# itailang/SampleNet

Measured on AMD Instinct MI355X. Metric: point-clouds/sec fwd+bwd, Bx1024->64 soft-proj+Chamfer, higher is better.
Workload: dtype f32; 1 GPU; BASELINE configs[1]: SampleNet sampler train step (fwd + simplification/projection losses + bwd), B=32 per GPU, 1024->64 points, K=8, bottleneck 128; no optimizer step; batch_per_gpu=32, global_batch=32, n_in=1024, n_out=64, group_size=8, parallelism=dp1, rccl_ranks=0, grad_allreduce=none, execution=whole step replayed as one hipGraph

## Files before the change

### include/samplenet_hip_internal.h

```cpp
#ifndef SAMPLENET_HIP_INTERNAL_H
#define SAMPLENET_HIP_INTERNAL_H

#include "samplenet_hip.h"

#ifdef __cplusplus
extern "C" {
#endif

int sn_sampler_loss_forward(int nproj, const float *proj, const float *lsimp, const float *temperature,
                            float alpha, float lmbda, float min_sigma, float *loss, sn_stream_t stream);
int sn_sampler_loss_backward(int nproj, const float *grad_loss, const float *temperature, float alpha, float lmbda,
                             float min_sigma, float *grad_proj, float *grad_lsimp, float *grad_T, sn_stream_t stream);

int sn_pairscan_colmin_splits(int B, int N, int M);
int sn_pairscan_forward_partial(int B, int N, int M, int K, const float *P, int p_layout, const float *Q, int q_layout,
                                int *knn_idx, float *dist_q, int *idx_q, float *proj, int proj_layout,
                                const float *temperature, float min_sigma, void *workspace, long long workspace_bytes,
                                sn_stream_t stream);
int sn_pairscan_forward_partial_fc(int B, int N, int M, int K, const float *P, int p_layout, const float *fc_z,
                                   const float *fc_scale, const float *fc_shift, const float *fc_w, const float *fc_bias,
                                   int Kfc, float *q_out, int *knn_idx, float *dist_q, int *idx_q, float *proj,
                                   int proj_layout, const float *temperature, float min_sigma, void *workspace,
                                   long long workspace_bytes, sn_stream_t stream);
int sn_sampler_step_loss_forward(int B, int M, int N, int G, const float *dist_q, const void *colmin_ws, const float *proj,
                                 const float *temperature, float alpha, float lmbda, float weight, float min_sigma,
                                 float *dist_p, int *idx_p, int *argmax1, float *partial, float *loss, int defer_value,
                                 sn_stream_t stream);
int sn_sampler_step_loss_forward_direct(int B, int M, int N, const float *dist_q, const float *dist_p, const float *proj,
                                        const float *temperature, float alpha, float lmbda, float weight, float min_sigma,
                                        int *argmax1, float *partial, float *loss, int defer_value, sn_stream_t stream);
int sn_sampler_step_loss_backward(int B, int N, int M, int K, const float *P, int p_layout, const float *Q,
                                  const int *knn_idx, const int *idx_q, const int *idx_p, const int *argmax1,
                                  const float *temperature, float min_sigma, float alpha, float lmbda, float weight,
                                  const float *grad_loss, float *grad_Q, float *gsig_scratch, float *grad_T,
                                  const float *deferred_partial, float *deferred_loss, sn_stream_t stream);
int sn_pairscan_forward_keys(int B, int N, int M, int K, const float *P, int p_layout, float *Q, const float *fc_z,
                             const float *fc_scale, const float *fc_shift, const float *fc_w, const float *fc_bias, int Kfc,
                             int *knn_idx, float *dist_q, int *idx_q, float *proj, int proj_layout, const float *temperature,
                             float min_sigma, void *colmin_keys, float *qpart, void *qmax, sn_stream_t stream);
int sn_sampler_step_loss_keys(int B, int N, int M, int K, const float *P, int p_layout, const float *Q, const int *knn_idx,
                              const int *idx_q, void *colmin_keys, const float *qpart, const void *qmax, int G,
                              const float *temperature, float min_sigma, float alpha, float lmbda, float weight,
                              const float *grad_loss, float *grad_Q, float *gsig_scratch, float *grad_T, float *dpsum,
                              float *loss, sn_stream_t stream, void *deferred_tail, const float *grad_proj,
                              const float *grad_sigma);
int sn_surface_values_keys(int B, int N, int M, int G, const void *colmin_keys, const float *qpart, const void *qmax,
                           const float *temperature, float min_sigma, float weight, const float *y_bcn, float *simp_bnc,
                           float *dpsum, float *values, sn_stream_t stream);
int sn_surface_gather_upstream(int nproj, const float *g_lsimp, const float *g_sigma, const float *g_proj, float *scalars,
                               float *proj_out, sn_stream_t stream);
int sn_conv_stack_set_persist_min_tiles(int tiles);
int sn_fps_set_variant(int v);
int sn_step_tail_bytes(void);
int sn_step_tail_set_error_words(void *tail_blob, const void *fwd_sync, const void *bwd_sync);


int sn_layer_forward_bn(int R, int Ci, int Co, const float *ain, const float *coef_prev, const float *W,
                        const float *bias, float *z, float *stats, const float *gamma, const float *beta,
                        float eps, float momentum, float *running_mean, float *running_var,
                        long long *num_batches_tracked, float *coef, sn_stream_t stream);
int sn_conv_forward_bn_pool(int R, int Ci, int Co, int npts, const float *ain, const float *coef_prev, const float *W,
                            const float *bias, float *z, float *stats, const float *gamma, const float *beta, float eps,
                            float momentum, float *running_mean, float *running_var, long long *num_batches_tracked,
                            float *coef, float *pool_val, int *pool_idx, float *pooled, int *argsel, float *zsel,
                            sn_stream_t stream);
int sn_conv_stack_forward_supported(int B, int N, int nlayers, const int *channels);
long long sn_conv_stack_acc_elems(int nlayers);
int sn_conv_stack_z1_free_supported(int B, int N, int nlayers, const int *channels);
long long sn_conv_stack_acc_sum_elems(int nlayers, const int *channels);
int sn_conv_stack_forward_bn(int B, int N, int nlayers, const int *channels, const float *x, const float *const *W,
                             const float *const *bias, const float *const *gamma, const float *const *beta,
                             float *const *running_mean, float *const *running_var, long long *const *num_batches_tracked,
                             const float *eps, const float *momentum, float *const *z, float *const *coef, long long *acc,
                             float *pool_val, int *pool_idx, float *pooled, int *argsel, float *zsel, sn_stream_t stream);
long long sn_conv_stack_backward_scratch_floats(int B, int N, int nlayers, const int *channels);
int sn_conv_stack_backward(int B, int N, int nlayers, const int *channels, const float *x, const float *const *W,
                           const float *bias0, const float *const *z, const float *const *coef, const float *gsel,
                           const int *argsel, const float *kcoef_top, long long *acc, float *scratch, float *const *dW,
                           float *const *dgamma, float *const *dbeta, float *const *dbias, const void *step_tail,
                           sn_stream_t stream);
int sn_layer_backward(int R, int Ci, int Co, int dz_mode, const float *dy, const float *z, const float *kcoef,
                      const float *gsel, const int *argsel, int npts, const float *W, const float *zprev,
                      const float *coef_prev, float *dyprev, float *stats, float *part, float *dW, float *db,
                      float *prev_dgamma, float *prev_dbeta, float *prev_dbias, float *prev_kcoef, long long prev_bn_rows,
                      sn_stream_t stream);
long long sn_layer_backward_in3_stats_floats(int R, int Ci, int Co);
int sn_layer_backward_in3(int R, int Ci, int Co, const float *dy, const float *z, const float *kcoef, const float *W,
                          const float *zprev, const float *coef_prev, float *stats, float *part, float *dW,
                          float *prev_dgamma, float *prev_dbeta, float *prev_dbias, float *prev_kcoef, const float *x_in,
                          const float *W_in, const float *b_in, float *dW_in, sn_stream_t stream);

int sn_fc_chain_forward_supported(int R, int C0, int H, int nl);
int sn_fc_chain_forward(int R, int C0, int H, int nl, const float *a0, const float *const *W, const float *const *bias,
                        const float *const *gamma, const float *const *beta, float *const *running_mean,
                        float *const *running_var, long long *const *num_batches_tracked, const float *eps,
                        const float *momentum, float *const *z, float *const *coef, float *xbuf, unsigned *sync,
                        sn_stream_t stream);
int sn_fc_chain_forward_pool_supported(int B, int N, int C0, int H, int nl);
int sn_fc_chain_forward_pool(int B, int N, int nconv, long long *acc, const float *pool_val, const int *pool_idx,
                             const float *gamma5, const float *beta5, float *running_mean5, float *running_var5,
                             long long *num_batches_tracked5, float eps5, float momentum5, float *coef5, float *pooled,
                             int *argsel, float *zsel, int H, int nl, const float *const *W, const float *const *bias,
                             const float *const *gamma, const float *const *beta, float *const *running_mean,
                             float *const *running_var, long long *const *num_batches_tracked, const float *eps,
                             const float *momentum, float *const *z, float *const *coef, float *xbuf, unsigned *sync,
                             sn_stream_t stream);
int sn_fc_chain_forward_pool_out_supported(int B, int N, int C0, int H, int nl, int Co);
int sn_fc_chain_forward_pool_out(int B, int N, int nconv, long long *acc, const float *pool_val, const int *pool_idx,
                                 const float *gamma5, const float *beta5, float *running_mean5, float *running_var5,
                                 long long *num_batches_tracked5, float eps5, float momentum5, float *coef5, float *pooled,
                                 int *argsel, float *zsel, int H, int nl, const float *const *W, const float *const *bias,
                                 const float *const *gamma, const float *const *beta, float *const *running_mean,
                                 float *const *running_var, long long *const *num_batches_tracked, const float *eps,
                                 const float *momentum, float *const *z, float *const *coef, float *xbuf, unsigned *sync, int Co,
                                 const float *Wo, const float *bo, const float *gamma_o, const float *beta_o, float *running_mean_o,
                                 float *running_var_o, long long *num_batches_tracked_o, float eps_o, float momentum_o, float *zo,
                                 float *coef_o, float *y, sn_stream_t stream);
int sn_fc_chain_backward_supported(int R, int ns, const int *Co, const int *Ci);
int sn_fc_chain_backward(int R, int ns, const int *Co, const int *Ci, const float *gy, const float *const *W,
                         const float *const *zprev, const float *const *coefprev, const long long *bn_rows,
                         float *const *dgamma, float *const *dbeta, float *const *dbias, float *const *dW, float *db_top,
                         const float *const *aprev, const int *araw, float *gout, float *kout, float *xbuf,
                         unsigned *sync, sn_stream_t stream);
int sn_fc_chain_backward_obn(int R, int ns, const int *Co, const int *Ci, const float *gy, const float *zo, const float *coef_o, int fixed,
                             float *dgamma_o, float *dbeta_o, const float *const *W, const float *const *zprev,
                             const float *const *coefprev, const long long *bn_rows, float *const *dgamma, float *const *dbeta,
                             float *const *dbias, float *const *dW, float *db_top, const float *const *aprev, const int *araw, float *gout,
                             float *kout, float *xbuf, unsigned *sync, sn_stream_t stream);
int sn_bn_batch_stats_twopass(int R, int C, const float *z, const float *gamma, const float *beta, float eps, float momentum,
                              float *running_mean, float *running_var, long long *num_batches_tracked, float *coef,
                              sn_stream_t stream);

int sn_layer_forward_bn_out(int R, int Ci, int Co, const float *ain, const float *coef_prev, const float *W, const float *bias,
                            float *z, const float *gamma, const float *beta, float eps, float momentum, float *running_mean,
                            float *running_var, long long *num_batches_tracked, float *coef, float *y, sn_stream_t stream);
int sn_bn_output_forward(int R, int C, int training, const float *z, const float *gamma, const float *beta, float eps,
                         float momentum, float *running_mean, float *running_var, long long *num_batches_tracked, float *coef,
                         float *y, sn_stream_t stream);
int sn_bn_output_backward(int R, int C, int fixed, const float *gy, const float *z, const float *coef, float *dz, float *dgamma,
                          float *dbeta, sn_stream_t stream);

int sn_pool_backward_bn(int B, int C, long long R, const float *g, const float *pooled, const float *zsel, float *gsel,
                        const float *coef, float *dgamma, float *dbeta, float *dbias, float *kcoef, sn_stream_t stream);

int sn_linear_backward(int R, int Ci, int Co, int dz_mode, const float *dy, const float *z, const float *kcoef,
                       const float *gsel, const int *argsel, int npts, const float *W, const float *zprev,
                       const float *coef_prev, float *dyprev, float *stats, float *part, float *dW, sn_stream_t stream);

int sn_conv_backward_partials(int R, int Ci, int Co, int dz_mode, const float *dy, const float *z, const float *kcoef,
                              const float *gsel, const int *argsel, int npts, const float *W, const float *zprev,
                              const float *coef_prev, float *dyprev, float *stats, float *part, sn_stream_t stream);

int sn_linear_forward_maxpool_supported(int R, int Ci, int Co, int npts);
int sn_linear_forward_maxpool(int R, int Ci, int Co, int npts, const float *ain, const float *coef_prev, const float *W,
                              const float *bias, float *z, unsigned long long *keys, float *pooled, int *argsel, float *zsel,
                              int keys_cleared, sn_stream_t stream);

int sn_linear_forward_maxpool_wide_supported(int R, int Ci, int Co, int npts);
long long sn_linear_forward_maxpool_wide_scratch_bytes(int R, int Ci, int Co, int npts);
int sn_linear_forward_maxpool_wide(int R, int Ci, int Co, int npts, const float *ain, const float *coef_prev, const float *W,
                                   const float *bias, float *z, void *scratch, float *pooled, int *argsel, float *zsel,
                                   void *wplanes, int planes_ready, sn_stream_t stream);
int sn_pool_dgrad_sparse_supported(int B, int npts, int Ci, int Co);
// ... 112 lines not shown
```

### samplenet_amd/_lib.py

```python
import ctypes
import os

import torch

_HERE = os.path.dirname(os.path.abspath(__file__))
LIB_PATH = os.environ.get("SAMPLENET_AMD_LIB") or os.path.join(_HERE, "lib", "libsamplenet_hip.so")

_vp = ctypes.c_void_p
_i = ctypes.c_int
_f = ctypes.c_float

PROTOTYPES = {
    "sn_abi_version": [],
    "sn_last_error_string": [],
    "sn_workspace_bytes": [ctypes.c_char_p, _i, _i, _i, _i],
    "sn_pairscan_forward": [_i, _i, _i, _i, _vp, _i, _vp, _i, _vp, _vp, _vp, _vp, _vp, _vp, _vp, _i, _vp, _vp, _f, _vp],
    "sn_pairscan_workspace_bytes": [_i, _i, _i],
    "sn_pairscan_forward_ws": [_i, _i, _i, _i, _vp, _i, _vp, _i, _vp, _vp, _vp, _vp, _vp, _vp, _vp, _i, _vp, _vp, _f, _vp,
                               ctypes.c_longlong, _vp],
    "sn_soft_bwd_splits": [_i, _i],
    "sn_sigma_grad": [_i, _vp, _vp, _f, _vp, _vp],
    "sn_sigma_forward": [_vp, _f, _vp, _vp],
    "sn_chamfer_forward": [_i, _i, _vp, _i, _vp, _vp, _vp, _vp, _vp, _vp],
    "sn_chamfer_backward": [_i, _i, _vp, _i, _vp, _vp, _vp, _vp, _vp, _vp, _vp, _vp],
    "sn_simplification_loss_forward": [_i, _i, _i, _vp, _vp, _f, _vp, _vp, _vp, _vp],
    "sn_simplification_loss_backward": [_i, _i, _vp, _i, _vp, _vp, _vp, _vp, _f, _vp, _vp, _vp, _i, _vp],
    "sn_chamfer_mean_loss_forward": [_i, _i, _i, _vp, _vp, _vp, _vp, _vp, _vp],
    "sn_chamfer_mean_loss_backward": [_i, _i, _vp, _i, _vp, _vp, _vp, _vp, _vp, _vp, _vp],
    "sn_pcrnet_head_forward": [_i, _vp, _vp, _vp, _vp, _vp],
    "sn_pcrnet_head_backward": [_i, _vp, _vp, _vp, _vp, _vp, _vp],
    "sn_pcrnet_head_rot_forward": [_i, _i, _vp, _vp, _vp, _vp, _vp, _vp, _vp],
    "sn_pcrnet_head_rot_backward": [_i, _i, _vp, _vp, _vp, _vp, _vp, _vp, _vp, _vp, _vp, _vp],
    "sn_sampler_loss_forward": [_i, _vp, _vp, _vp, _f, _f, _f, _vp, _vp],
    "sn_sampler_loss_backward": [_i, _vp, _vp, _f, _f, _f, _vp, _vp, _vp, _vp],
    "sn_pairscan_colmin_splits": [_i, _i, _i],
    "sn_pairscan_forward_partial": [_i, _i, _i, _i, _vp, _i, _vp, _i, _vp, _vp, _vp, _vp, _i, _vp, _f, _vp, ctypes.c_longlong, _vp],
    "sn_pairscan_forward_partial_fc": [_i, _i, _i, _i, _vp, _i, _vp, _vp, _vp, _vp, _vp, _i, _vp, _vp, _vp, _vp, _vp, _i, _vp, _f,
                                       _vp, ctypes.c_longlong, _vp],
    "sn_sampler_step_loss_forward": [_i, _i, _i, _i, _vp, _vp, _vp, _vp, _f, _f, _f, _f, _vp, _vp, _vp, _vp, _vp, _i, _vp],
    "sn_sampler_step_loss_forward_direct": [_i, _i, _i, _vp, _vp, _vp, _vp, _f, _f, _f, _f, _vp, _vp, _vp, _i, _vp],
    "sn_sampler_step_loss_backward": [_i, _i, _i, _i, _vp, _i, _vp, _vp, _vp, _vp, _vp, _vp, _f, _f, _f, _f, _vp, _vp, _vp,
                                      _vp, _vp, _vp, _vp],
    "sn_pairscan_forward_keys": [_i, _i, _i, _i, _vp, _i, _vp, _vp, _vp, _vp, _vp, _vp, _i, _vp, _vp, _vp, _vp, _i, _vp, _f, _vp, _vp,
                                 _vp, _vp],
    "sn_sampler_step_loss_keys": [_i, _i, _i, _i, _vp, _i, _vp, _vp, _vp, _vp, _vp, _vp, _i, _vp, _f, _f, _f, _f, _vp, _vp, _vp, _vp,
                                  _vp, _vp, _vp, _vp, _vp, _vp],
    "sn_surface_values_keys": [_i, _i, _i, _i, _vp, _vp, _vp, _vp, _f, _f, _vp, _vp, _vp, _vp, _vp],
    "sn_surface_gather_upstream": [_i, _vp, _vp, _vp, _vp, _vp, _vp],
    "sn_conv_stack_set_persist_min_tiles": [_i],
    "sn_conv_stack_set_in3_blocks": [_i],
    "sn_step_tail_bytes": [],
    "sn_step_tail_set_error_words": [_vp, _vp, _vp],
    "sn_prefix_point_minima": [_i, _i, _i, _i, _vp, _vp, _vp, _vp, _vp, _vp],
    "sn_prefix_simplification_loss_forward": [_i, _i, _i, _i, _vp, _vp, _vp, _vp, _vp, _vp, _vp, _vp],
    "sn_prefix_simplification_loss_backward": [_i, _i, _i, _i, _vp, _vp, _vp, _vp, _vp, _vp, _vp, _vp, _vp, _vp],
    "sn_prefix_pack": [_i, _i, _i, _i, _vp, _vp, _vp, _vp],
    "sn_chamfer_forward_valid": [_i, _i, _vp, _i, _vp, _vp, _i, _vp, _vp, _vp, _vp, _vp, ctypes.c_longlong, _vp],
    "sn_pcrnet_head_rot_forward_grouped": [_i, _i, _i, _vp, _vp, _vp, _vp, _vp, _vp, _vp],
    "sn_pcrnet_head_rot_backward_grouped": [_i, _i, _i, _vp, _vp, _vp, _vp, _vp, _vp, _vp, _vp, _vp],
    "sn_chamfer_mean_loss_forward_grouped": [_i, _i, _i, _i, _i, _vp, _vp, _vp, _vp, _vp, _vp],
    "sn_chamfer_mean_loss_backward_grouped": [_i, _i, _vp, _i, _vp, _i, _i, _vp, _vp, _vp, _vp, _vp, _vp, _vp],
    "sn_cyclic_pad_cat": [_i, _i, _i, _i, _vp, _vp, _vp, _vp],
    "sn_cyclic_pad_cat_backward": [_i, _i, _i, _i, _vp, _vp, _vp, _vp],
    "sn_prefix_scatter_sum": [_i, _i, _i, _i, _vp, _vp, _vp, _vp],
    "sn_knn": [_i, _i, _i, _i, _vp, _i, _vp, _i, _vp, _vp, _vp],
    "sn_nn_matching": [_i, _i, _i, _vp, _i, _vp, _i, _vp, _vp],
    "sn_furthest_point_sample": [_i, _i, _i, _vp, _i, _vp, _vp, _vp],
    "sn_fps_set_variant": [_i],
    "sn_qrot_forward": [_i, _i, _vp, _vp, _vp, _vp],
    "sn_qrot_backward": [_i, _i, _vp, _vp, _vp, _vp, _vp, _vp],
    "sn_group_point": [_i, _i, _i, _i, _i, _vp, _vp, _vp, _vp],
    "sn_group_point_grad": [_i, _i, _i, _i, _i, _vp, _vp, _vp, _vp],
    "sn_grouping_operation": [_i, _i, _i, _i, _i, _vp, _vp, _vp, _vp],
    "sn_grouping_operation_grad": [_i, _i, _i, _i, _i, _vp, _vp, _vp, _vp],
    "sn_soft_weights_forward": [_i, _i, _i, _i, _vp, _vp, _vp, _vp, _f, _vp, _vp],
    "sn_soft_weights_backward": [_i, _i, _i, _i, _vp, _vp, _vp, _vp, _f, _vp, _vp, _vp, _vp, _vp, _vp],
    "sn_weighted_gather_forward": [_i, _i, _i, _i, _i, _vp, _vp, _vp, _vp, _vp],
    "sn_weighted_gather_backward": [_i, _i, _i, _i, _i, _vp, _vp, _vp, _vp, _vp, _vp, _vp],
    "sn_soft_project_backward": [_i, _i, _i, _i, _vp, _i, _vp, _i, _vp, _vp, _f, _vp, _i, _vp, _i, _vp, _vp, _vp],
    "sn_soft_project_backward_ordered": [_i, _i, _i, _i, _vp, _i, _vp, _i, _vp, _vp, _f, _vp, _i, _vp, _i, _vp, _vp, _vp, _vp],
    "sn_soft_weights_backward_ordered": [_i, _i, _i, _i, _vp, _vp, _vp, _vp, _f, _vp, _vp, _vp, _vp, _vp, _vp, _vp],
    "sn_weighted_gather_backward_ordered": [_i, _i, _i, _i, _i, _vp, _vp, _vp, _vp, _vp, _vp, _vp, _vp],
    "sn_linear_stats_blocks": [_i],
    "sn_layer_forward_bn": [_i, _i, _i, _vp, _vp, _vp, _vp, _vp, _vp, _vp, _vp, _f, _f, _vp, _vp, _vp, _vp, _vp],
    "sn_conv_forward_bn_pool": [_i, _i, _i, _i, _vp, _vp, _vp, _vp, _vp, _vp, _vp, _vp, _f, _f, _vp, _vp, _vp, _vp, _vp, _vp,
                                _vp, _vp, _vp, _vp],
    "sn_layer_backward": [_i, _i, _i, _i, _vp, _vp, _vp, _vp, _vp, _i, _vp, _vp, _vp, _vp, _vp, _vp, _vp, _vp, _vp, _vp, _vp,
                          _vp, ctypes.c_longlong, _vp],
    "sn_conv_stack_forward_supported": [_i, _i, _i, _vp],
    "sn_conv_stack_acc_elems": [_i],
    "sn_conv_stack_z1_free_supported": [_i, _i, _i, _vp],
    "sn_conv_stack_acc_sum_elems": [_i, ctypes.c_void_p],
    "sn_conv_stack_backward_scratch_floats": [_i, _i, _i, _vp],
    "sn_conv_stack_backward": [_i, _i, _i] + [_vp] * 17,
    "sn_conv_stack_forward_bn": [_i, _i, _i] + [_vp] * 20,
    "sn_layer_backward_in3_stats_floats": [_i, _i, _i],
    "sn_layer_backward_in3": [_i, _i, _i] + [_vp] * 17 + [_vp],
    "sn_linear_forward": [_i, _i, _i, _vp, _vp, _vp, _vp, _vp, _vp, _vp],
    "sn_linear_forward_rows": [_i, _i, _i, _vp, _vp, _vp, _vp, _vp, _vp],
    "sn_bn_finalize": [_i, _i, ctypes.c_longlong, _vp, _vp, _vp, _f, _f, _vp, _vp, _vp, _vp, _vp],
    "sn_fc_chain_forward_supported": [_i, _i, _i, _i],
    "sn_fc_chain_forward_pool_supported": [_i, _i, _i, _i, _i],
    "sn_fc_chain_forward_pool": [_i, _i, _i, _vp, _vp, _vp, _vp, _vp, _vp, _vp, _vp, _f, _f, _vp, _vp, _vp, _vp, _i, _i] + [_vp] * 14,
    "sn_fc_chain_forward_pool_out_supported": [_i, _i, _i, _i, _i, _i],
    "sn_fc_chain_forward_pool_out": [_i, _i, _i, _vp, _vp, _vp, _vp, _vp, _vp, _vp, _vp, _f, _f, _vp, _vp, _vp, _vp, _i, _i] + [_vp] * 13 +
                                    [_i, _vp, _vp, _vp, _vp, _vp, _vp, _vp, _f, _f, _vp, _vp, _vp, _vp],
    "sn_fc_chain_forward": [_i, _i, _i, _i, _vp, _vp, _vp, _vp, _vp, _vp, _vp, _vp, _vp, _vp, _vp, _vp, _vp, _vp, _vp],
    "sn_fc_chain_backward_supported": [_i, _i, _vp, _vp],
    "sn_fc_chain_backward": [_i, _i, _vp, _vp, _vp, _vp, _vp, _vp, _vp, _vp, _vp, _vp, _vp, _vp, _vp, _vp, _vp, _vp, _vp, _vp, _vp],
    "sn_fc_chain_backward_obn": [_i, _i, _vp, _vp, _vp, _vp, _vp, _i, _vp, _vp] + [_vp] * 16,
    "sn_linear_forward_maxpool_supported": [_i, _i, _i, _i],
    "sn_linear_forward_maxpool": [_i, _i, _i, _i, _vp, _vp, _vp, _vp, _vp, _vp, _vp, _vp, _vp, _i, _vp],
    "sn_linear_forward_maxpool_wide_supported": [_i, _i, _i, _i],
    "sn_linear_forward_maxpool_wide_scratch_bytes": [_i, _i, _i, _i],
    "sn_linear_forward_maxpool_wide": [_i, _i, _i, _i, _vp, _vp, _vp, _vp, _vp, _vp, _vp, _vp, _vp, _vp, _i, _vp],
    "sn_pointnet_narrow_forward_supported": [_i, _i, _i, _i, _i],
    "sn_pointnet_narrow_forward": [_i, _vp, _vp, _vp, _vp, _vp, _vp, _vp, _vp, _vp, _vp, _i, _vp, _vp, _vp, _vp, _vp, _i, _vp],
    "sn_pointnet_narrow_backward_supported": [_i, _i, _i, _i, _i],
    "sn_pointnet_narrow_backward": [_i, _vp, _vp, _vp, _vp, _vp, _vp, _vp, _vp, _vp, _i, _vp, _vp],
    "sn_cloud_transform_forward": [_i, _i, _i, _vp, _vp, _vp, _vp],
    "sn_cloud_transform_backward": [_i, _i, _i, _vp, _vp, _vp, _vp, _vp, _vp],
    "sn_orthogonality_loss_forward": [_i, _i, _vp, _vp, _vp, _vp],
    "sn_orthogonality_loss_backward": [_i, _i, _vp, _vp, _vp, _vp],
    "sn_bn_relu_forward": [ctypes.c_longlong, _i, _vp, _vp, _vp, _vp],
    "sn_bn_relu_backward": [ctypes.c_longlong, _i, _vp, _vp, _vp, _i, _vp, _vp],
    "sn_skinny_linear_supported": [_i, _i, _i],
    "sn_skinny_linear_scratch_bytes": [_i, _i, _i],
    "sn_skinny_linear": [_i, _i, _i, _vp, _vp, _vp, _i, _vp, _i, _vp, _vp, _vp, _vp],
    "sn_skinny_linear2": [_i, _i, _i, _vp, _vp, _i, _vp, _vp, _i, _vp, _i, _vp, _vp, _i, _vp, _vp, _vp],
    "sn_skinny_wgrad": [_i, _i, _i, _vp, _vp, _i, _vp, _vp, _vp, _vp, _vp],
    "sn_pool_dgrad_sparse_supported": [_i, _i, _i, _i],
    "sn_pool_dgrad_sparse": [_i, _i, _i, _i, _vp, _vp, _vp, _vp, _vp, _vp, _vp, _vp],
    "sn_bn_batch_stats_twopass": [_i, _i, _vp, _vp, _vp, _f, _f, _vp, _vp, _vp, _vp, _vp],
    "sn_bn_eval_coef": [_i, _vp, _vp, _f, _vp, _vp, _vp, _vp],
    "sn_layer_forward_bn_out": [_i, _i, _i, _vp, _vp, _vp, _vp, _vp, _vp, _vp, _f, _f, _vp, _vp, _vp, _vp, _vp, _vp],
    "sn_bn_output_forward": [_i, _i, _i, _vp, _vp, _vp, _f, _f, _vp, _vp, _vp, _vp, _vp, _vp],
    "sn_bn_output_backward": [_i, _i, _i, _vp, _vp, _vp, _vp, _vp, _vp, _vp],
    "sn_pool_forward": [_i, _i, _i, _vp, _vp, _vp, _vp, _vp, _vp],
    "sn_pool_backward": [_i, _i, _vp, _vp, _vp, _vp, _vp, _vp],
    "sn_pool_backward_bn": [_i, _i, ctypes.c_longlong, _vp, _vp, _vp, _vp, _vp, _vp, _vp, _vp, _vp, _vp],
    "sn_bn_backward_coef": [_i, _i, ctypes.c_longlong, _vp, _vp, _vp, _vp, _vp, _vp, _vp],
    "sn_linear_dgrad": [_i, _i, _i, _i, _vp, _vp, _vp, _vp, _vp, _i, _vp, _vp, _vp, _vp, _vp, _vp],
    "sn_linear_backward": [_i, _i, _i, _i, _vp, _vp, _vp, _vp, _vp, _i, _vp, _vp, _vp, _vp, _vp, _vp, _vp, _vp],
    "sn_conv_backward_partials": [_i, _i, _i, _i, _vp, _vp, _vp, _vp, _vp, _i, _vp, _vp, _vp, _vp, _vp, _vp, _vp],
    "sn_linear_wgrad_splits": [_i, _i, _i, _i],
    "sn_linear_wgrad": [_i, _i, _i, _i, _vp, _vp, _vp, _vp, _vp, _i, _vp, _vp, _vp, _vp, _vp, _vp],
    "sn_approxmatch": [_i, _i, _i, _vp, _vp, _vp, _vp, _vp],
    "sn_matchcost": [_i, _i, _i, _vp, _vp, _vp, _vp, _vp, _vp],
    "sn_matchcost_grad": [_i, _i, _i, _vp, _vp, _vp, _vp, _vp, _vp],
    "sn_emd_loss": [_i, _i, _i, _vp, _vp, _vp, _vp, _vp, _vp, _vp],
    "sn_emd_loss_fast": [_i, _i, _i, _vp, _vp, _vp, _vp, _vp, _vp, _vp],
    "sn_emd_set_sweep2d": [_i],
    "sn_emd_set_segments": [_i],
    "sn_adam_chunk_elems": [],
    "sn_adam_state_bytes": [],
    "sn_adam_update": [_i, _vp, _vp, _vp, _vp, ctypes.c_double, ctypes.c_double, ctypes.c_double, ctypes.c_double,
                       ctypes.c_double, _i, _vp],
    "sn_pose_error_forward": [_i, _vp, _vp, _vp, _vp, _vp, _vp, _vp],
    "sn_pose_error_backward": [_i, _vp, _vp, _vp, _vp, _vp, _vp, _vp],
    "sn_chamfer_mean_per_cloud": [_i, _i, _i, _vp, _vp, _vp, _vp],
    "sn_batch_state_bytes": [],
    "sn_batch_assemble": [_i, _i, _i, _i, _i, _vp, _vp, _vp, ctypes.c_ulonglong, _i, _i, ctypes.c_longlong, _vp, _vp, _i, _vp, _vp,
                          _vp, _vp, _vp, _vp],
}
_RESTYPES = {"sn_last_error_string": ctypes.c_char_p, "sn_workspace_bytes": ctypes.c_longlong,
             "sn_pairscan_workspace_bytes": ctypes.c_longlong, "sn_linear_forward_maxpool_wide_scratch_bytes": ctypes.c_longlong,
             "sn_skinny_linear_scratch_bytes": ctypes.c_longlong,
             "sn_adam_state_bytes": ctypes.c_longlong,
             "sn_batch_state_bytes": ctypes.c_longlong,
             "sn_layer_backward_in3_stats_floats": ctypes.c_longlong,
             "sn_conv_stack_acc_elems": ctypes.c_longlong,
             "sn_conv_stack_acc_sum_elems": ctypes.c_longlong,
             "sn_conv_stack_backward_scratch_floats": ctypes.c_longlong}


class SampleNetHipError(RuntimeError):
    pass


def _load():
    if not os.path.exists(LIB_PATH):
        raise ImportError(
            "samplenet_amd: %s not found. Build it with `python samplenet_amd/build.py` (hipcc, gfx950). "
            "There is no CPU / eager fallback." % LIB_PATH)
    lib = ctypes.CDLL(LIB_PATH)
    for name, argtypes in PROTOTYPES.items():
        try:
            fn = getattr(lib, name)
        except AttributeError as e:
            raise ImportError("samplenet_amd: %s does not export %s (stale build?)" % (LIB_PATH, name)) from e
        fn.argtypes = argtypes
        fn.restype = _RESTYPES.get(name, _i)
    return lib


lib = _load()
if lib.sn_abi_version() != 1:
    raise ImportError("samplenet_amd: ABI version mismatch in %s" % LIB_PATH)


def check(rc, what=""):
    if rc != 0:
        msg = lib.sn_last_error_string()
        raise SampleNetHipError("%s failed (code %d): %s" % (what or "samplenet_hip call", rc, (msg or b"").decode()))


def ptr(t):
    return None if t is None else t.data_ptr()


try:
    from torch._C import _cuda_getCurrentRawStream as _raw_stream
except ImportError:
    _raw_stream = None


def stream_of(t):
    if _raw_stream is not None:
        return _raw_stream(t.device.index if t.device.index is not None else torch.cuda.current_device())
    return torch.cuda.current_stream(t.device).cuda_stream
```

### samplenet_amd/csrc/pointnet_mlp.hip

```cpp
#include "mlp_host.h"

namespace sn {

template <class T, bool FULL, int AMODE, int KT = 0, bool PLANES = false, bool IN3A = false>
__global__ void __launch_bounds__(T::THREADS) __attribute__((amdgpu_waves_per_eu(T::THREADS / 128, 8))) linear_fwd_kernel(FwdArgs g)
{
    extern __shared__ __attribute__((aligned(16))) float lds[];
    SN_TL(0);
    SN_TL_ID(0);
    const int row0 = blockIdx.x * T::BM, col0 = blockIdx.y * T::BN;
    const int R = g.a.rows, Co = g.w.co, Ci = g.w.ci;
    f32x16 acc[T::TM][T::TN];
#pragma unroll
    for (int i = 0; i < T::TM; ++i)
#pragma unroll
        for (int j = 0; j < T::TN; ++j)
#pragma unroll
            for (int e = 0; e < 16; ++e) acc[i][j][e] = 0.f;
    const ActSrc a = g.a;
    const WSrc w = g.w;
    const int lane = threadIdx.x & 63;
    const int wave = __builtin_amdgcn_readfirstlane(threadIdx.x >> 6);
    const int wr = wave / T::WC, wc = wave % T::WC;
    float biasv[T::TN];
// ... 795 lines not shown
            w.x *= mw, w.y *= mw, w.z *= mw, w.w *= mw;
            *reinterpret_cast<float4 *>(Ws + r * LD + c4) = w;
        }
    __syncthreads();
    f32x16 acc0, acc1;
#pragma unroll
    for (int e = 0; e < 16; ++e) acc0[e] = 0.f, acc1[e] = 0.f;
    const int kph = Ci / 8, kb = wave * (Ci / 4) + h * kph;
    const float *ap0 = As + l31 * LD + kb, *ap1 = As + (32 + l31) * LD + kb, *bp = Ws + l31 * LD + kb;
    for (int t = 0; t < kph; t += 4) {
        const float4 a0 = *reinterpret_cast<const float4 *>(ap0 + t), a1 = *reinterpret_cast<const float4 *>(ap1 + t);
        const float4 b = *reinterpret_cast<const float4 *>(bp + t);
        acc0 = __builtin_amdgcn_mfma_f32_32x32x2f32(a0.x, b.x, acc0, 0, 0, 0);
        acc1 = __builtin_amdgcn_mfma_f32_32x32x2f32(a1.x, b.x, acc1, 0, 0, 0);
        acc0 = __builtin_amdgcn_mfma_f32_32x32x2f32(a0.y, b.y, acc0, 0, 0, 0);
        acc1 = __builtin_amdgcn_mfma_f32_32x32x2f32(a1.y, b.y, acc1, 0, 0, 0);
        acc0 = __builtin_amdgcn_mfma_f32_32x32x2f32(a0.z, b.z, acc0, 0, 0, 0);
        acc1 = __builtin_amdgcn_mfma_f32_32x32x2f32(a1.z, b.z, acc1, 0, 0, 0);
        acc0 = __builtin_amdgcn_mfma_f32_32x32x2f32(a0.w, b.w, acc0, 0, 0, 0);
        acc1 = __builtin_amdgcn_mfma_f32_32x32x2f32(a1.w, b.w, acc1, 0, 0, 0);
    }
    wave_sum_to_wave0(acc0, red);
    wave_sum_to_wave0(acc1, red + 3 * 16 * 64);
    if (wave != 0) return;
    float s0 = 0.f;
    const bool vec_out = Co % 32 == 0;
#pragma unroll
    for (int s2 = 0; s2 < 2; ++s2)
#pragma unroll
        for (int e = 0; e < 16; ++e) {
            const int row = 32 * s2 + frag_row(e, lane);
            const float v = (s2 ? acc1[e] : acc0[e]) + bias;
            if (row < R && colok) {
                s0 += v;
                if (!vec_out) g.z[(size_t)row * Co + col] = v;
            }
            Ts[row * 36 + l31] = v;
        }
    if (vec_out) {
#pragma unroll
        for (int i = 0; i < 8; ++i) {
            const int row = 8 * i + (lane >> 3);
            const float4 v = *reinterpret_cast<const float4 *>(Ts + row * 36 + (lane & 7) * 4);
            if (row < R) *reinterpret_cast<float4 *>(g.z + (size_t)row * Co + col0 + (lane & 7) * 4) = v;
        }
    }
    s0 += __shfl_xor(s0, 32);
    if (g.bn.coef) {
        if (blockIdx.x == 0 && lane == 0 && g.bn.num_batches_tracked) *g.bn.num_batches_tracked += 1;
        const float meanf = s0 / (float)g.bn.R;
        float s2v = 0.f;
#pragma unroll
        for (int s2 = 0; s2 < 2; ++s2)
#pragma unroll
            for (int e = 0; e < 16; ++e) {
                const float d = ((s2 ? acc1[e] : acc0[e]) + bias) - meanf;
                if (32 * s2 + frag_row(e, lane) < R && colok) s2v += d * d;
            }
        s2v += __shfl_xor(s2v, 32);
        if (lane < 32 && colok) {
            const double rR = fast_rcp((double)g.bn.R);
            const double mean = (double)s0 * rR;
            const double dm = mean - (double)meanf;
            double var = (double)s2v * rR - dm * dm;
            if (var < 0.0) var = 0.0;
            const float invstd = (float)fast_rsqrt(var + (double)g.bn.eps);
            const float sc = bn_g * invstd;
            g.bn.coef[col] = sc;
            g.bn.coef[Co + col] = bn_b - (float)mean * sc;
            g.bn.coef[2 * Co + col] = (float)mean;
            g.bn.coef[3 * Co + col] = invstd;
            if (g.bn.running_mean) {
                const double unbiased = g.bn.R > 1 ? var * (double)g.bn.R * fast_rcp((double)(g.bn.R - 1)) : var;
                g.bn.running_mean[col] = (1.f - g.bn.momentum) * bn_rm + g.bn.momentum * (float)mean;
                g.bn.running_var[col] = (1.f - g.bn.momentum) * bn_rv + g.bn.momentum * (float)unbiased;
            }
        }
    }
}

struct WSplitJob {
    const float *w[4];
    __bf16 *dst[4];
    int elems[4];
    int first[5];
    int n;
    unsigned long long *zero_keys;
    int nkeys;
};
__device__ __forceinline__ void wsplit_block(const WSplitJob &job, int blk, int tid)
{
    int l = 0;
#pragma unroll
    for (int q = 1; q < 4; ++q)
        if (q < job.n && blk >= job.first[q]) l = q;
    const int e = (blk - job.first[l]) * 1024 + tid * 4;
    if (e >= job.elems[l]) return;
    const float4 v = *reinterpret_cast<const float4 *>(job.w[l] + e);
    bf16x4 p1, p2, p3;
    const float f[4] = {v.x, v.y, v.z, v.w};
#pragma unroll
    for (int t = 0; t < 4; ++t) {
        __bf16 h1, h2, h3;
        split3(f[t], h1, h2, h3);
        p1[t] = h1, p2[t] = h2, p3[t] = h3;
    }
    __bf16 *d = job.dst[l] + e;
    *reinterpret_cast<bf16x4 *>(d) = p1;
    *reinterpret_cast<bf16x4 *>(d + job.elems[l]) = p2;
    *reinterpret_cast<bf16x4 *>(d + 2 * (size_t)job.elems[l]) = p3;
}

__global__ void __launch_bounds__(256) conv_in3_fwd_kernel(int R, int Co, const float *__restrict__ x,
                                                           const float *__restrict__ W, const float *__restrict__ bias,
                                                           float *__restrict__ z, float *__restrict__ stats,
                                                           long long *__restrict__ acc_out = nullptr,
                                                           long long *__restrict__ clear_flags = nullptr, WSplitJob job = WSplitJob{},
                                                           int nb = 1)
{
    if (job.n > 0 && blockIdx.y == 0 && (int)blockIdx.x < job.first[job.n]) wsplit_block(job, blockIdx.x, threadIdx.x);
    if (job.zero_keys && blockIdx.y == 0) {
        const int i = blockIdx.x * 256 + threadIdx.x;
        if (i < job.nkeys) job.zero_keys[i] = 0ull;
    }
    if (clear_flags && blockIdx.x == 0 && blockIdx.y == 0 && threadIdx.x == 0) clear_flags[0] = 0;
    __shared__ float red[2][16][64];
    const int q = threadIdx.x & 15, rs = threadIdx.x >> 4;
    const int cl = q * 4, co = blockIdx.y * 64 + cl;
    const bool vec = (Co & 3) == 0 && co + 3 < Co;
    float w[4][3], b[4];
#pragma unroll
    for (int j = 0; j < 4; ++j) {
        const int c = min(co + j, Co - 1);
        const float m = co + j < Co ? 1.f : 0.f;
        w[j][0] = W[c * 3 + 0] * m, w[j][1] = W[c * 3 + 1] * m, w[j][2] = W[c * 3 + 2] * m;
        b[j] = bias ? bias[c] * m : 0.f;
    }
    const int nblocks = (R + 63) / 64;
    const int blk0 = blockIdx.x * nb, blk1 = min(blk0 + nb, nblocks);
    long long fx0 = 0, fx1 = 0;
    for (int blk = blk0; blk < blk1; ++blk) {
        const int row0 = blk * 64;
        float xs[4][3];
#pragma unroll
        for (int i = 0; i < 4; ++i) {
            const int r = min(row0 + rs + 16 * i, R - 1);
            xs[i][0] = x[(size_t)r * 3], xs[i][1] = x[(size_t)r * 3 + 1], xs[i][2] = x[(size_t)r * 3 + 2];
        }
        float s0[4] = {0.f, 0.f, 0.f, 0.f}, s1[4] = {0.f, 0.f, 0.f, 0.f};
#pragma unroll
        for (int i = 0; i < 4; ++i) {
            const int r = row0 + rs + 16 * i;
            const float m = r < R ? 1.f : 0.f;
            float v[4];
#pragma unroll
            for (int j = 0; j < 4; ++j) {
                v[j] = (fmaf(w[j][2], xs[i][2], fmaf(w[j][1], xs[i][1], w[j][0] * xs[i][0])) + b[j]) * m;
                s0[j] += v[j];
                s1[j] += v[j] * v[j];
            }
            if (r < R && z) {
                if (vec) {
                    buf_store4<SN_ST_Z>(make_float4(v[0], v[1], v[2], v[3]), make_rsrc(z + (size_t)row0 * Co, (unsigned)(min(64, R - row0) * Co) * 4),
                                        (unsigned)((rs + 16 * i) * Co + co) * 4, 0u);
                } else {
#pragma unroll
                    for (int j = 0; j < 4; ++j)
                        if (co + j < Co) z[(size_t)r * Co + co + j] = v[j];
                }
            }
        }
        if (blk > blk0) __syncthreads();
#pragma unroll
        for (int j = 0; j < 4; ++j) red[0][rs][cl + j] = s0[j], red[1][rs][cl + j] = s1[j];
        __syncthreads();
        if (threadIdx.x < 64 && (stats || acc_out)) {
            const int c = blockIdx.y * 64 + threadIdx.x;
            if (c < Co) {
                float a0 = 0.f, a1 = 0.f;
#pragma unroll
                for (int k = 0; k < 16; ++k) a0 += red[0][k][threadIdx.x], a1 += red[1][k][threadIdx.x];
                if (acc_out) {
                    if (nb == 1) {
                        fx_add<kFxShiftFwd>(acc_out, blockIdx.x % kFxSlots, 0, c, a0);
                        fx_add<kFxShiftFwd>(acc_out, blockIdx.x % kFxSlots, 1, c, a1);
                    } else {
                        fx_local_add<kFxShiftFwd>(fx0, acc_out, 0, c, a0);
                        fx_local_add<kFxShiftFwd>(fx1, acc_out, 1, c, a1);
                    }
                } else {
                    float *st = stats + (size_t)blk * 2 * Co;
                    st[c] = a0;
                    st[Co + c] = a1;
// ... 446 lines not shown
        SN_LAUNCH_CHECK();
        return 0;
    }
    if (R <= 32) {
        g.bn = bn;
        g.stats = nullptr;
    }
    if (coef_prev)
        launch_fwd<ACT_BN_RELU>(g, st);
    else
        launch_fwd<ACT_NONE>(g, st);
    if (R > 32)
        hipLaunchKernelGGL(bn_finalize_kernel, dim3((Co + kChan - 1) / kChan), dim3(1024), 0, st, sn_linear_stats_blocks(R), Co, stats, bn);
    SN_LAUNCH_CHECK();
    return 0;
}

extern "C" int sn_conv_forward_bn_pool(int R, int Ci, int Co, int npts, const float *ain, const float *coef_prev, const float *W,
                                       const float *bias, float *z, float *stats, const float *gamma, const float *beta,
                                       float eps, float momentum, float *running_mean, float *running_var,
                                       long long *num_batches_tracked, float *coef, float *pool_val, int *pool_idx,
                                       float *pooled, int *argsel, float *zsel, sn_stream_t stream)
{
    SN_REQUIRE(R >= 1 && Ci >= 1 && Co >= 1 && npts >= 1, "bad size");
    SN_REQUIRE(ain && W && z && stats && gamma && beta && coef && pool_val && pool_idx && pooled && argsel && zsel && coef_prev,
               "null pointer");
    if (R <= 64 || R % 64 || npts % 64 || R % npts || Co % 64 || Ci % 64)
        return sn_set_error(SN_ERR_UNSUPPORTED, "sn_conv_forward_bn_pool: needs 64-aligned rows / points / channels");
    FwdArgs g{};
    g.a = make_act(ain, coef_prev, R, Ci);
    g.w.w = W, g.w.co = Co, g.w.ci = Ci;
    g.bias = bias, g.z = z, g.stats = stats;
    g.pool_val = pool_val, g.pool_idx = pool_idx, g.pool_npts = npts;
    const BnFwd bn{gamma, beta, running_mean, running_var, num_batches_tracked, coef, eps, momentum, (long long)R};
    hipStream_t st = (hipStream_t)stream;
    launch_fwd<ACT_BN_RELU>(g, st);
    hipLaunchKernelGGL(bn_finalize_pool_kernel, dim3((Co + kChan - 1) / kChan), dim3(1024), 0, st, sn_linear_stats_blocks(R), Co,
                       stats, bn, R / npts, npts / 64, pool_val, pool_idx, pooled, argsel, zsel);
    SN_LAUNCH_CHECK();
    return 0;
}

extern "C" int sn_conv_stack_forward_supported(int B, int N, int nlayers, const int *channels)
{
    if (B < 1 || N < 1 || nlayers < 2 || !channels || channels[0] != 3) return 0;
    const long long R = (long long)B * N;
    if (R <= 64 || R > (1ll << 30) || N % 64) return 0;
    bool wide = false;
    long long nb = 0;
    for (int l = 1; l <= nlayers; ++l) {
        if (channels[l] % 64 || channels[l] > 2 * kFxRow) return 0;
        wide = wide || channels[l] > 128;
        if (l < nlayers) nb += ((long long)channels[l] * channels[l + 1] + 1023) / 1024;
    }
    if (wide && (!SN_BF16X3 || nlayers - 1 > 4 || nb > R / 64 || channels[nlayers] > 128 || channels[1] > 128)) return 0;
    return 1;
}

[[maybe_unused]] constexpr long long kWPlaneLL = (long long)128 * 128 * 3 * 2 / 8;
[[maybe_unused]] constexpr long long kWPlaneWideLL = (long long)256 * 256 * 3 * 2 / 8;
static bool conv_stack_wide(int nlayers, const int *channels)
{
    for (int l = 1; l <= nlayers; ++l)
        if (channels[l] > kFxRow) return true;
    return false;
}
extern "C" int sn_conv_stack_z1_free_supported(int B, int N, int nlayers, const int *channels)
{
#if SN_BF16X3
    if (!sn_conv_stack_forward_supported(B, N, nlayers, channels) || nlayers < 3 || nlayers - 1 > 4) return 0;
    if (channels[1] != 64 || channels[2] != 64) return 0;
    long long nb = 0;
    for (int l = 1; l < nlayers; ++l) nb += ((long long)channels[l] * channels[l + 1] + 1023) / 1024;
    return nb <= (long long)B * N / 64 ? 1 : 0;
#else
    return 0;
#endif
}
extern "C" long long sn_conv_stack_acc_sum_elems(int nlayers, const int *channels)
{
    if (nlayers <= 0) return 0;
    return (long long)nlayers * ((channels && conv_stack_wide(nlayers, channels)) ? 2 : 1) * kFxLayer;
}
extern "C" long long sn_conv_stack_acc_elems(int nlayers)
{
    return nlayers > 0 ? (long long)nlayers * 2 * kFxLayer + (long long)(nlayers - 1) * kWPlaneWideLL : 0;
}

static int g_persist_min_tiles = 4;
static int g_in3_blocks = 0;
extern "C" int sn_conv_stack_set_in3_blocks(int blocks)
{
    const int prev = g_in3_blocks;
    g_in3_blocks = blocks < 0 ? 0 : blocks;
    return prev;
}
extern "C" int sn_conv_stack_set_persist_min_tiles(int tiles)
{
    const int old = g_persist_min_tiles;
    g_persist_min_tiles = tiles;
    return old;
}
template <class TT, int KT, bool IN3A>
static int launch_fwd_persist(const FwdArgs &g, int ntiles, int tpw, int nwg, hipStream_t st)
{
    const size_t lds = sizeof(float) * ((size_t)(KT / BKX) * 3 * TT::BM * LDX + 2 * KT + (size_t)2 * TT::WR * 2 * TT::BN + (size_t)TT::WR * TT::WC * 16 * 36);
    static SnLdsAttr attr;
    if (sn_lds_attr(attr, (const void *)linear_fwd_persist_kernel<TT, KT, IN3A, 2>, lds, "linear_fwd_persist_kernel")) return SN_ERR_UNSUPPORTED;
    hipLaunchKernelGGL((linear_fwd_persist_kernel<TT, KT, IN3A, 2>), dim3(nwg), dim3(TT::THREADS), lds, st, g, ntiles, tpw);
    return 0;
}

extern "C" int sn_conv_stack_forward_bn(int B, int N, int nlayers, const int *channels, const float *x, const float *const *W,
                                        const float *const *bias, const float *const *gamma, const float *const *beta,
                                        float *const *running_mean, float *const *running_var,
                                        long long *const *num_batches_tracked, const float *eps, const float *momentum,
                                        float *const *z, float *const *coef, long long *acc, float *pool_val, int *pool_idx,
                                        float *pooled, int *argsel, float *zsel, sn_stream_t stream)
{
    if (!sn_conv_stack_forward_supported(B, N, nlayers, channels))
        return sn_set_error(SN_ERR_UNSUPPORTED, "sn_conv_stack_forward_bn: needs N % 64 == 0 and 64 / 128 (/ 256 inside the stack) channels");
    SN_REQUIRE(x && W && gamma && beta && eps && momentum && z && coef && acc && pool_val && pool_idx, "null pointer");
    SN_REQUIRE((pooled && argsel && zsel) || (!pooled && !argsel && !zsel), "pooled / argsel / zsel: all or none");
    hipStream_t st = (hipStream_t)stream;
    const int R = B * N;
    const bool wide = conv_stack_wide(nlayers, channels);
    const size_t S = wide ? 2 * (size_t)kFxLayer : (size_t)kFxLayer;
    SN_REQUIRE(!wide || pooled, "a stack with a layer above 128 channels finishes its own pool (the FC chain's pool stage reads the 128-channel layout)");
    auto bn_of = [&](int l) {
        return BnFwd{gamma[l], beta[l], running_mean ? running_mean[l] : nullptr, running_var ? running_var[l] : nullptr,
                     num_batches_tracked ? num_batches_tracked[l] : nullptr, coef[l], eps[l], momentum[l], (long long)R};
    };
    for (int l = 0; l < nlayers; ++l) SN_REQUIRE(W[l] && gamma[l] && beta[l] && (z[l] || l == 0) && coef[l], "null pointer");
    const bool z1free = z[0] == nullptr;
#if !SN_BF16X3
    SN_REQUIRE(!z1free, "z[0] == NULL needs the split-bf16 build");
#endif
    SN_REQUIRE(!z1free || (channels[1] == 64 && channels[2] == 64), "z[0] == NULL: 3 -> 64 -> 64 channels only");
    WSplitJob job{};
    __bf16 *planes[8] = {nullptr};
#if SN_BF16X3
    if (nlayers - 1 <= 4) {
        __bf16 *base = reinterpret_cast<__bf16 *>(acc + (size_t)nlayers * S);
        int nb = 0;
        for (int l = 1; l < nlayers; ++l) {
            const int li = l - 1, el = channels[l] * channels[l + 1];
            planes[l] = base + (size_t)li * (wide ? kWPlaneWideLL : kWPlaneLL) * 4;
            job.w[li] = W[l], job.dst[li] = planes[l], job.elems[li] = el, job.first[li] = nb;
            nb += (el + 1023) / 1024;
        }
        job.n = nlayers - 1, job.first[job.n] = nb;
        if (nb > R / 64) job.n = 0;
    }
#endif
    const bool keys_pool = !pooled || (B > 32 && N >= 128 && channels[nlayers] <= 128);
    if (keys_pool) {
        job.zero_keys = reinterpret_cast<unsigned long long *>(pool_val), job.nkeys = B * 2 * channels[nlayers];
        SN_REQUIRE((long long)job.nkeys <= (long long)(R / 64) * 256, "too few rows to clear the pool keys");
    }
    int in3_nb = 1;
    {
        const long long need = std::max<long long>(job.n > 0 ? job.first[job.n] : 0, keys_pool ? (job.nkeys + 255) / 256 : 0);
        while (in3_nb < 8 && (R / 64) / (in3_nb * 2) >= std::max<long long>(need, 4 * device_cus()) && (R / 64) % (in3_nb * 2) == 0) in3_nb *= 2;
        if (g_in3_blocks > 0 && (R / 64) / g_in3_blocks >= std::max<long long>(need, 1)) in3_nb = g_in3_blocks;
    }
    hipLaunchKernelGGL(conv_in3_fwd_kernel, dim3((R / 64 + in3_nb - 1) / in3_nb, channels[1] / 64), dim3(256), 0, st, R, channels[1], x, W[0],
                       bias ? bias[0] : nullptr, z[0], (float *)nullptr, acc, acc + (size_t)(nlayers - 1) * S + kFxPoison, job,
                       in3_nb);
    using T = TileBig;
    for (int l = 1; l < nlayers; ++l) {
        const int Ci = channels[l], Co = channels[l + 1];
        FwdArgs g{};
        g.a = make_act(z[l - 1], nullptr, R, Ci);
        g.w.w = W[l], g.w.co = Co, g.w.ci = Ci;
        g.bias = bias ? bias[l] : nullptr, g.z = z[l], g.stats = nullptr;
        g.acc_in = acc + (size_t)(l - 1) * S, g.bn_prev = bn_of(l - 1), g.acc_out = acc + (size_t)l * S;
        if (l >= 2) g.zero_ptr = acc + (size_t)(l - 2) * S, g.zero_n = (int)S;
        if (l == nlayers - 1) {
            g.pool_npts = N;
            if (!keys_pool) g.pool_val = pool_val, g.pool_idx = pool_idx;
            else g.pool_keys = reinterpret_cast<unsigned long long *>(pool_val);
        }
        g.wplanes = job.n > 0 ? planes[l] : nullptr;
        const bool pl = g.wplanes != nullptr;
#if SN_BF16X3
        if (pl && g.z && (l < nlayers - 1 || keys_pool) && (l > 1 || z1free) && (Ci == 64 || Co == 128) && Ci <= 128 && Co <= 128 && R % 64 == 0) {
            const int ntiles = R / 64, per_cu = Co == 128 ? 1 : 2, nmax = device_cus() * per_cu;
            if (g_persist_min_tiles > 0 && ntiles >= g_persist_min_tiles * nmax) {
                const int tpw = (ntiles + nmax - 1) / nmax, nwg = (ntiles + tpw - 1) / tpw;
                if (l == 1) g.x3 = x, g.w3 = W[0], g.b3 = bias ? bias[0] : nullptr;
                int rc = 0;
                const bool ht = Co == 128 && l != 1;
                const int nmax_h = device_cus() * 2, tpw_h = 2 * ((ntiles + nmax_h - 1) / nmax_h), nwg_h = (2 * ntiles + tpw_h - 1) / tpw_h;
                using THT = Tile<32, 128, 1, 4>;
                if (l == 1) rc = launch_fwd_persist<T, 64, true>(g, ntiles, tpw, nwg, st);
                else if (ht && Ci == 128) rc = launch_fwd_persist<THT, 128, false>(g, 2 * ntiles, tpw_h, nwg_h, st);
                else if (ht) rc = launch_fwd_persist<THT, 64, false>(g, 2 * ntiles, tpw_h, nwg_h, st);
                else rc = launch_fwd_persist<T, 64, false>(g, ntiles, tpw, nwg, st);
                if (rc) return rc;
                continue;
            }
        }
#endif
        if (l == 1 && z1free) {
            SN_REQUIRE(pl, "z[0] == NULL: the weight planes are missing");
            g.x3 = x, g.w3 = W[0], g.b3 = bias ? bias[0] : nullptr;
            const dim3 grid(R / T::BM, Co / T::BN);
            const size_t lds = shaped_lds(lds_bytes<T>() + (size_t)2 * Ci * sizeof(float), grid);
            hipLaunchKernelGGL((linear_fwd_kernel<T, true, ACT_BN_RELU_FX, 64, SN_BF16X3 != 0, SN_BF16X3 != 0>), grid, dim3(T::THREADS), lds, st, g);
            continue;
        }
        if (Co % 128 == 0) {
            using TW = TileWide;
            const dim3 grid(R / TW::BM, Co / TW::BN);
            const size_t lds = shaped_lds(lds_bytes<TW>() + (size_t)2 * Ci * sizeof(float), grid);
#define SN_FWD_FX(TT, KT_)                                                                                                \
    do {                                                                                                                  \
        if (pl) hipLaunchKernelGGL((linear_fwd_kernel<TT, true, ACT_BN_RELU_FX, KT_, SN_BF16X3 != 0>), grid, dim3(TT::THREADS), lds, st, g); \
        else hipLaunchKernelGGL((linear_fwd_kernel<TT, true, ACT_BN_RELU_FX, KT_>), grid, dim3(TT::THREADS), lds, st, g);  \
    } while (0)
            if (Ci == 256) {
                SN_REQUIRE(pl, "a 256-channel input needs the pre-split weight planes");
                hipLaunchKernelGGL((linear_fwd_kernel<TW, true, ACT_BN_RELU_FX, 256, SN_BF16X3 != 0>), grid, dim3(TW::THREADS), lds, st, g);
            } else if (Ci == 128 && pl) SN_FWD_FX(TW, 128);
            else if (Ci == 128) SN_FWD_FX(TW, 0);
            else SN_FWD_FX(TW, 64);
            continue;
        }
        const dim3 grid(R / T::BM, Co / T::BN);
        const size_t lds = shaped_lds(lds_bytes<T>() + (size_t)2 * Ci * sizeof(float), grid);
        if (Ci == 128 && pl) SN_FWD_FX(T, 128);
// ... 127 lines not shown
```

### samplenet_amd/csrc/pointnet_mlp_backward.hip

```cpp
#include "mlp_host.h"

namespace sn {

struct DgradArgs {
    DzSrc dz;
    WSrc w;
    ActSrc prev;
    float *dyprev;
    float *stats;
    BnBwd bb;
};

template <class T, bool FULL, int ZMODE, int PMODE>
__device__ __forceinline__ void dgrad_body(const DgradArgs &g, int bx, int by, float *lds)
{
    SN_TL(0);
    SN_TL_ID(2);
    const int row0 = bx * T::BM, col0 = by * T::BN;
    const int R = g.dz.rows, Co = g.w.co, Ci = g.w.ci;
    f32x16 acc[T::TM][T::TN];
#pragma unroll
    for (int i = 0; i < T::TM; ++i)
#pragma unroll
        for (int j = 0; j < T::TN; ++j)
// ... 72 lines not shown
    int rows_per_split;
    int ncols;
};

template <class T, bool FULL, int ZMODE, int PMODE>
__device__ __forceinline__ void wgrad_body(const WgradArgs &g, int bx, int by, int bz, float *lds)
{
    SN_TL(0);
    SN_TL_ID(1);
    const int m0 = bx * T::BM, n0 = by * T::BN;
    const int Co = g.dz.ch, Ce = g.ncols;
    const int r0 = bz * g.rows_per_split;
    const int r1 = min(g.dz.rows, r0 + g.rows_per_split);
    f32x16 acc[T::TM][T::TN];
#pragma unroll
    for (int i = 0; i < T::TM; ++i)
#pragma unroll
        for (int j = 0; j < T::TN; ++j)
#pragma unroll
            for (int e = 0; e < 16; ++e) acc[i][j][e] = 0.f;
    DzSrc dz = g.dz;
    ActSrc pv = g.prev;
    dz.rows = r1;
    pv.rows = r1;
    gemm_tile<T, false, false>(
        acc, max(0, r1 - r0), [&](int x, int k) { return dz.template load_c4<FULL, ZMODE>(r0 + k, m0 + x); },
        [&](int x, int k) { return pv.template load_c4<FULL, PMODE>(r0 + k, n0 + x); }, lds);

    const int lane = threadIdx.x & 63;
    const int wave = __builtin_amdgcn_readfirstlane(threadIdx.x >> 6);
    const int wr = wave / T::WC, wc = wave % T::WC;
    float *P = g.part + (size_t)bz * Co * Ce;
#pragma unroll
    for (int j = 0; j < T::TN; ++j) {
        const int col = n0 + (wc * T::TN + j) * 32 + (lane & 31);
#pragma unroll
        for (int i = 0; i < T::TM; ++i)
#pragma unroll
            for (int e = 0; e < 16; ++e) {
                const int row = m0 + (wr * T::TM + i) * 32 + frag_row(e, lane);
                if (FULL || (row < Co && col < Ce)) P[(size_t)row * Ce + col] = acc[i][j][e];
            }
    }
    SN_TL(3);
    SN_TL_DRAIN();
    SN_TL(5);
}

template <class T, bool FULL, int ZMODE, int PMODE>
__global__ void __launch_bounds__(T::THREADS) linear_wgrad_kernel(WgradArgs g)
{
    extern __shared__ __attribute__((aligned(16))) float lds[];
    wgrad_body<T, FULL, ZMODE, PMODE>(g, blockIdx.x, blockIdx.y, blockIdx.z, lds);
}

template <class T, int ZMODE, int PMODE>
__global__ void __launch_bounds__(T::THREADS) linear_bwd_kernel(DgradArgs d, WgradArgs w, int n_w, int wgx, int wgy, int dgx)
{
    extern __shared__ __attribute__((aligned(16))) float lds[];
    const int id = blockIdx.x;
    if (id < n_w) {
        wgrad_body<T, true, ZMODE, PMODE>(w, id % wgx, (id / wgx) % wgy, id / (wgx * wgy), lds);
    } else {
        const int e = id - n_w;
        dgrad_body<T, true, ZMODE, PMODE>(d, e % dgx, e / dgx, lds);
    }
}

struct ConvBwdArgs {
    DzSrc dz;
    const float *W;
    const float *zprev, *scale_prev, *shift_prev;
    float *dyprev, *stats, *part;
    int ntiles;
    const float *xin;
    const float *w_in, *b_in;
    const long long *acc_in;
    BnBwd bb_in;
    long long *acc_out;
    long long *zero_ptr;
    int zero_n;
    int part_wg_stride, part_ld, stats_ld;
    const float *dyacc;
};

__device__ __forceinline__ float4 buf_load4(sn_rsrc r, unsigned voff, unsigned soff)
{
    const u32x4 x = __builtin_amdgcn_raw_buffer_load_b128(r, voff, soff, 0);
    return make_float4(__uint_as_float(x.x), __uint_as_float(x.y), __uint_as_float(x.z), __uint_as_float(x.w));
}
typedef unsigned u32x3 __attribute__((ext_vector_type(3)));
__device__ __forceinline__ float4 buf_load3(sn_rsrc r, unsigned voff, unsigned soff)
{
    const u32x3 x = __builtin_amdgcn_raw_buffer_load_b96(r, voff, soff, 0);
    return make_float4(__uint_as_float(x.x), __uint_as_float(x.y), __uint_as_float(x.z), 0.f);
}
__device__ __forceinline__ int4 buf_load4i(sn_rsrc r, unsigned voff, unsigned soff)
{
    const u32x4 x = __builtin_amdgcn_raw_buffer_load_b128(r, voff, soff, 0);
    return make_int4((int)x.x, (int)x.y, (int)x.z, (int)x.w);
}
__device__ __forceinline__ float buf_load1(sn_rsrc r, unsigned voff, unsigned soff)
{
    return __uint_as_float(__builtin_amdgcn_raw_buffer_load_b32(r, voff, soff, 0));
}

struct CbfRsrc {
    sn_rsrc z, dy, zprev, dyprev, argsel, gsel, dyacc;
};

template <int CO, int CI, int TR, int ZMODE, int NZ4, int NP4, bool SKIP_P = false, int GZ = CO, int GP = CI>
__device__ __forceinline__ void cbf_issue_loads(const CbfRsrc &rs, int tile, int b, unsigned zvo, unsigned pvo, unsigned avo,
                                                float4 (&rz)[NZ4], float4 (&rdy)[NZ4], float4 (&rp)[NP4], int4 &rag,
                                                float4 &rgs)
{
    constexpr int ZSTEP = 256 / (CO / 4), PSTEP = 256 / (CI / 4);
    const unsigned zso = (unsigned)tile * (TR * GZ * 4), pso = (unsigned)tile * (TR * GP * 4);
#pragma unroll
    for (int q = 0; q < NZ4; ++q) {
        rz[q] = buf_load4(rs.z, zvo, zso + q * (ZSTEP * GZ * 4));
        if (ZMODE == DZ_BN) rdy[q] = buf_load4(rs.dy, zvo, zso + q * (ZSTEP * GZ * 4));
    }
#pragma unroll
    for (int q = 0; q < (SKIP_P ? 0 : NP4); ++q) rp[q] = buf_load4(rs.zprev, pvo, pso + q * (PSTEP * GP * 4));
    if (ZMODE == DZ_POOL) {
        rag = buf_load4i(rs.argsel, avo, (unsigned)b * (CO * 4));
        rgs = buf_load4(rs.gsel, avo, (unsigned)b * (CO * 4));
    }
}

template <int CO, int CI, int TR, int ZMODE, bool FULLR, int NZ4, int NP4>
__device__ __forceinline__ void cbf_stage(const ConvBwdArgs &g, int tile, int n0, int tid, float *__restrict__ Zs,
                                          float *__restrict__ Ps,
                                          const float4 (&rz)[NZ4], const float4 (&rdy)[NZ4], const float4 (&rp)[NP4],
                                          const int4 &rag, const float4 &rgs, const float4 &k1, const float4 &k2,
                                          const float4 &k3, const float4 &sc4, const float4 &sh4)
{
    constexpr int ZSTEP = 256 / (CO / 4), PSTEP = 256 / (CI / 4);
    constexpr int LDZ = CO + 2, LDP = CI + 2;
    const int R = g.dz.rows;
    const int row0 = tile * TR;
    const int zc4 = (tid % (CO / 4)) * 4, zr = tid / (CO / 4);
    const int pc4 = (tid % (CI / 4)) * 4, pr = tid / (CI / 4);
#pragma unroll
    for (int q = 0; q < NZ4; ++q) {
        const int rt = zr + q * ZSTEP;
        float4 d;
        if (ZMODE == DZ_POOL) {
            const int n = n0 + rt;
            d.x = rag.x == n ? rgs.x : 0.f;
            d.y = rag.y == n ? rgs.y : 0.f;
            d.z = rag.z == n ? rgs.z : 0.f;
            d.w = rag.w == n ? rgs.w : 0.f;
        } else {
            d = rdy[q];
        }
        float4 v = make_float4(fmaf(k1.x, d.x, fmaf(k2.x, rz[q].x, k3.x)), fmaf(k1.y, d.y, fmaf(k2.y, rz[q].y, k3.y)),
                               fmaf(k1.z, d.z, fmaf(k2.z, rz[q].z, k3.z)), fmaf(k1.w, d.w, fmaf(k2.w, rz[q].w, k3.w)));
        if (!FULLR) {
            const float m = row0 + rt < R ? 1.f : 0.f;
            v.x *= m, v.y *= m, v.z *= m, v.w *= m;
        }
        float *o = Zs + rt * LDZ + zc4;
        *reinterpret_cast<float2 *>(o) = make_float2(v.x, v.y);
        *reinterpret_cast<float2 *>(o + 2) = make_float2(v.z, v.w);
    }
// ... 365 lines not shown
#pragma unroll
        for (int k = 0; k < NST; ++k) {
            float a = red[k * CI + tid];
            if (RB == 2) a += red[(NST + k) * CI + tid];
            if (!IN3 && g.acc_out)
                fx_add<kFxShiftBwd>(g.acc_out, blockIdx.x % kFxSlots, k, tid, a);
            else
                st[k * CI + tid] = a;
        }
        if (IN3) st[5 * CI + tid] = tid < 9 ? red[RB * NST * CI + tid] : 0.f;
    }
    SN_TL_DRAIN();
    SN_TL(7);
}

typedef short s16x4 __attribute__((ext_vector_type(4)));
typedef short s16x8 __attribute__((ext_vector_type(8)));
typedef __attribute__((address_space(3))) s16x4 lds_s16x4;
__device__ __forceinline__ bf16x8 lds_tr8(const __bf16 *p, int pitch)
{
    const s16x4 lo = __builtin_amdgcn_ds_read_tr16_b64_v4i16((lds_s16x4 *)(p));
    const s16x4 hi = __builtin_amdgcn_ds_read_tr16_b64_v4i16((lds_s16x4 *)(p + 4 * pitch));
    const s16x8 v = {lo[0], lo[1], lo[2], lo[3], hi[0], hi[1], hi[2], hi[3]};
    return __builtin_bit_cast(bf16x8, v);
}

__device__ __forceinline__ bf16x8 lds_tr8_2(const __bf16 *plo, const __bf16 *phi)
{
    const s16x4 lo = __builtin_amdgcn_ds_read_tr16_b64_v4i16((lds_s16x4 *)(plo));
    const s16x4 hi = __builtin_amdgcn_ds_read_tr16_b64_v4i16((lds_s16x4 *)(phi));
    const s16x8 v = {lo[0], lo[1], lo[2], lo[3], hi[0], hi[1], hi[2], hi[3]};
    return __builtin_bit_cast(bf16x8, v);
}

template <int CI, int CO>
struct CbxShape {
    static constexpr int TR = CO == 128 ? 32 : 64;
    static constexpr int KS = (CI == 64 && CO == 128) ? 2 : 1;
    static constexpr bool SWZ = CO == 128;
    static constexpr int LDZ = SWZ ? 160 : CO + 8, LDP = SWZ ? (CI == 128 ? 160 : 96) : CI + 8;
    static constexpr int ZPL = TR * LDZ, PPL = TR * LDP;
    static constexpr int BUF = 3 * (ZPL + PPL);
    static constexpr int TSZ = 4 * 32 * 36;
    static constexpr int XSZ = 2 * 3 * TR;
    static constexpr size_t TOFF = (size_t)2 * BUF * 2;
    static constexpr size_t LDS_BYTES = TOFF + TSZ * sizeof(float);
    static constexpr size_t LDS_BYTES_IN3 = LDS_BYTES + (XSZ + 4 * CI) * sizeof(float);
    static_assert(LDS_BYTES_IN3 <= 160 * 1024, "tile buffers exceed the LDS");
};

template <int CO, int CI, int TR, int ZMODE, bool FULLR, int NZ4>
__device__ __forceinline__ void cbx_stage(const ConvBwdArgs &g, int tile, int n0, int tid, __bf16 *__restrict__ Zb,
                                          const float4 (&rz)[NZ4], const float4 (&rdy)[NZ4], const int4 &rag, const float4 &rgs,
                                          const float4 &k1, const float4 &k2, const float4 &k3)
{
    constexpr int ZSTEP = 256 / (CO / 4);
    constexpr int LDZ = CbxShape<CI, CO>::LDZ;
    const int R = g.dz.rows;
    const int row0 = tile * TR;
    const int zc4 = (tid % (CO / 4)) * 4, zr = tid / (CO / 4);
#pragma unroll
    for (int q = 0; q < NZ4; ++q) {
        const int rt = zr + q * ZSTEP;
        float4 d;
        if (ZMODE == DZ_POOL) {
            const int n = n0 + rt;
            d.x = rag.x == n ? rgs.x : 0.f;
            d.y = rag.y == n ? rgs.y : 0.f;
            d.z = rag.z == n ? rgs.z : 0.f;
            d.w = rag.w == n ? rgs.w : 0.f;
        } else {
            d = rdy[q];
        }
        float4 v = make_float4(fmaf(k1.x, d.x, fmaf(k2.x, rz[q].x, k3.x)), fmaf(k1.y, d.y, fmaf(k2.y, rz[q].y, k3.y)),
                               fmaf(k1.z, d.z, fmaf(k2.z, rz[q].z, k3.z)), fmaf(k1.w, d.w, fmaf(k2.w, rz[q].w, k3.w)));
        if (!FULLR) {
            const float m = row0 + rt < R ? 1.f : 0.f;
            v.x *= m, v.y *= m, v.z *= m, v.w *= m;
        }
        stage_split_p<TR * LDZ, LDZ>(Zb, rt, CbxShape<CI, CO>::SWZ ? zc4 ^ (((rt >> 2) & 3) << 3) : zc4, v);
    }
}

template <int CI, int CO, int ZMODE, bool FULLR, bool IN3 = false, bool RZ1 = false, int GZ = CO, int GP = CI, int GW = CI, int DM = 0>
__global__ void __launch_bounds__(512) conv_bwd_bx3_kernel(ConvBwdArgs g)
{
    static_assert(DM == 0 || (!IN3 && CbxShape<CI, CO>::KS == 1), "two-pass modes: plain 128 x 128 tiles");
    static_assert(!RZ1 || IN3, "RZ1: the layer below must be the xyz layer");
    using S = CbxShape<CI, CO>;
    static_assert(!IN3 || (S::TR == 64 && ZMODE == DZ_BN), "IN3: 64-row tiles (one row per lane for the moments)");
    constexpr int NST = IN3 ? 5 : 2;
    constexpr int TR = S::TR, LDZ = S::LDZ, LDP = S::LDP, ZPL = S::ZPL, PPL = S::PPL, BUF = S::BUF;
    constexpr int NZ4 = TR * CO / 4 / 256, NP4 = TR * CI / 4 / 256;
    constexpr int NCB = CI / 32, NOB = CO / 32, RB = TR / 32;
    constexpr int KS = S::KS;
    constexpr bool kSkew = !IN3 && CI == 128 && CO == 128;
    constexpr int NDW = RB * NCB * KS;
    constexpr int NWT = NOB * NCB / 4;
    constexpr int KD = CO / 16 / KS, KW = TR / 16;
    static_assert((CI == 64 || CI == 128) && (CO == 64 || CO == 128), "instantiated for 64 / 128 channels");
    static_assert(NDW == 4 && NZ4 >= 1 && NP4 >= 1 && NWT >= 1, "wave roles below assume four dgrad waves per row tile");
    extern __shared__ __attribute__((aligned(16))) float lds[];
    __bf16 *Lb = reinterpret_cast<__bf16 *>(lds);
    float *Tf = reinterpret_cast<float *>(reinterpret_cast<char *>(lds) + S::TOFF);

    const int tid = threadIdx.x, lane = tid & 63, l31 = lane & 31, h = lane >> 5;
    const int wave = __builtin_amdgcn_readfirstlane(tid >> 6);
    float *Ts = Tf + (wave & 3) * (32 * 36);
    float *Xs = Tf + S::TSZ;
    const int R = g.dz.rows;
    const bool do_d = wave < 4;
    const int dwv = wave & 3;
    const int dt = dwv / KS, kh = dwv % KS;
    const int rb = dt % RB, cb = dt / RB;
    const int q0 = dwv * NWT;
    const int cob = q0 / NCB;
    const int G = gridDim.x;
    const int tile0 = blockIdx.x, tend = g.ntiles, tst = G;

    SN_TL(0);
#ifdef SN_TIMELINE
    sn_hw_record();
#endif
    if (do_d) {
        const int zc4 = (tid % (CO / 4)) * 4, pc4 = (tid % (CI / 4)) * 4;
        const bool fxin = ZMODE == DZ_BN && g.acc_in != nullptr;
        float4 k1 = make_float4(0.f, 0.f, 0.f, 0.f), k2 = k1, k3 = k1;
        if (!fxin) {
            k1 = *reinterpret_cast<const float4 *>(g.dz.k1 + zc4);
            k2 = *reinterpret_cast<const float4 *>(g.dz.k2 + zc4);
            k3 = *reinterpret_cast<const float4 *>(g.dz.k3 + zc4);
        }
        const float scd = g.scale_prev[cb * 32 + l31], shd = g.shift_prev[cb * 32 + l31];
        const unsigned qvo = ((rb * 32 + 4 * h) * GP + cb * 32 + l31) * 4;
        const unsigned ovo = ((rb * 32 + (lane >> 3)) * GP + cb * 32 + (lane & 7) * 4) * 4;
        const unsigned zvo = ((tid / (CO / 4)) * GZ + zc4) * 4, pvo = ((tid / (CI / 4)) * GP + pc4) * 4, avo = zc4 * 4;
        CbfRsrc rs;
        rs.z = make_rsrc(g.dz.z, (unsigned)R * GZ * 4);
        rs.dy = make_rsrc(ZMODE == DZ_BN ? g.dz.dy : g.dz.z, (unsigned)R * GZ * 4);
        rs.zprev = make_rsrc(g.zprev, (unsigned)R * GP * 4);
        rs.dyprev = make_rsrc(g.dyprev, (unsigned)R * GP * 4);
        rs.dyacc = make_rsrc(DM == 2 ? (const void *)g.dyacc : (const void *)g.zprev, (unsigned)R * GP * 4);
        const unsigned nclouds = ZMODE == DZ_POOL ? (unsigned)((R + g.dz.npts - 1) / g.dz.npts) : 1u;
        rs.argsel = make_rsrc(ZMODE == DZ_POOL ? (const void *)g.dz.argsel : (const void *)g.dz.z, nclouds * CO * 4);
        rs.gsel = make_rsrc(ZMODE == DZ_POOL ? (const void *)g.dz.gsel : (const void *)g.dz.z, nclouds * CO * 4);
        const sn_rsrc rsx = make_rsrc(IN3 ? (const void *)g.xin : (const void *)g.dz.z, (unsigned)R * 12);
        const bool xthr = IN3 && tid < 3 * TR / 4;
        int xslot[4];
#pragma unroll
        for (int j = 0; j < 4; ++j) {
            const int i = tid * 4 + j;
            xslot[j] = (i % 3) * TR + i / 3;
        }
        float4 rx = make_float4(0.f, 0.f, 0.f, 0.f);
        float gx0 = 0.f, gx1 = 0.f, gx2 = 0.f;
        float mom[9];
#pragma unroll
        for (int k = 0; k < 9; ++k) mom[k] = 0.f;
        const int tpc = ZMODE == DZ_POOL ? g.dz.npts / TR : 1;
        const int bstep = tst / tpc, tstep = tst - bstep * tpc;
        int cloud = tile0 / tpc, tic = tile0 - cloud * tpc;
        float4 rz[NZ4], rdy[NZ4], rp[NP4];
        int4 rag = make_int4(0, 0, 0, 0);
        float4 rgs = make_float4(0.f, 0.f, 0.f, 0.f);
        float s0 = 0.f, s1 = 0.f;
        float4 *W3s = reinterpret_cast<float4 *>(Xs + S::XSZ);
        if (RZ1 && tid < CI)
            W3s[tid] = make_float4(g.w_in[tid * 3], g.w_in[tid * 3 + 1], g.w_in[tid * 3 + 2], g.b_in ? g.b_in[tid] : 0.f);
        float4 vout[4];
#pragma unroll
        for (int i = 0; i < 4; ++i) vout[i] = make_float4(0.f, 0.f, 0.f, 0.f);

        int tile = tile0;
        cbf_issue_loads<CO, CI, TR, ZMODE, NZ4, NP4, true, GZ, GP>(rs, tile, cloud, zvo, pvo, avo, rz, rdy, rp, rag, rgs);
        if (xthr) rx = buf_load4(rsx, (unsigned)tid * 16, (unsigned)tile * (TR * 12));
        float wraw[KD][8];
#pragma unroll
        for (int kk = 0; kk < KD; ++kk)
#pragma unroll
            for (int t = 0; t < 8; ++t) wraw[kk][t] = g.W[(size_t)((kh * KD + kk) * 16 + 8 * h + t) * GW + cb * 32 + l31];
        if (fxin) {
            const float *Ks = Tf;
            __syncthreads();
            k1 = *reinterpret_cast<const float4 *>(Ks + zc4);
            k2 = *reinterpret_cast<const float4 *>(Ks + CO + zc4);
            k3 = *reinterpret_cast<const float4 *>(Ks + 2 * CO + zc4);
        }
        cbx_stage<CO, CI, TR, ZMODE, FULLR, NZ4>(g, tile, tic * TR, tid, Lb, rz, rdy, rag, rgs, k1, k2, k3);
        if (xthr) Xs[xslot[0]] = rx.x, Xs[xslot[1]] = rx.y, Xs[xslot[2]] = rx.z, Xs[xslot[3]] = rx.w;
        bf16x8 wf[KD][3];
#pragma unroll
        for (int kk = 0; kk < KD; ++kk)
#pragma unroll
            for (int t = 0; t < 8; ++t) {
                __bf16 h1, h2, h3;
                split3(wraw[kk][t], h1, h2, h3);
                wf[kk][0][t] = h1, wf[kk][1][t] = h2, wf[kk][2][t] = h3;
            }
        __syncthreads();
        for (int it = 0; tile < tend; ++it, tile += tst) {
            const __bf16 *Zb = Lb + (it & 1) * BUF;
            const auto store_prev = [&]() __attribute__((always_inline)) {
                if (!IN3 && it > 0 && kh == 0) {
                    const unsigned oso = (unsigned)(tile - tst) * (TR * GP * 4);
#pragma unroll
                    for (int i = 0; i < 4; ++i) buf_store4<SN_ST_DY>(vout[i], rs.dyprev, ovo, oso + i * (8 * GP * 4));
                }
            };
            store_prev();
            float zq[16], pq[16];
            if (!RZ1 && DM != 1 && (KS == 1 || kh == 0))
#pragma unroll
                for (int e = 0; e < 16; ++e)
                    zq[e] = buf_load1(rs.zprev, qvo, (unsigned)tile * (TR * GP * 4) + ((e & 3) + 8 * (e >> 2)) * (GP * 4));
            if (DM == 2)
#pragma unroll
                for (int e = 0; e < 16; ++e)
                    pq[e] = buf_load1(rs.dyacc, qvo, (unsigned)tile * (TR * GP * 4) + ((e & 3) + 8 * (e >> 2)) * (GP * 4));
            const bool more = tile + tst < tend;
            const int nxt = more ? tile + tst : tile;
            int ncloud = cloud, ntic = tic;
            if (more) {
                ncloud += bstep, ntic += tstep;
                if (ntic >= tpc) ntic -= tpc, ++ncloud;
            }
            cbf_issue_loads<CO, CI, TR, ZMODE, NZ4, NP4, true, GZ, GP>(rs, nxt, ncloud, zvo, pvo, avo, rz, rdy, rp, rag, rgs);
            if (xthr) rx = buf_load4(rsx, (unsigned)tid * 16, (unsigned)nxt * (TR * 12));
            __builtin_amdgcn_sched_barrier(0);
            if (it == 1) SN_TL(5);

            f32x16 acc;
#pragma unroll
            for (int e = 0; e < 16; ++e) acc[e] = 0.f;
            const int fsw = S::SWZ ? ((l31 >> 2) & 3) ^ h : 0;
            const __bf16 *apr = Zb + (rb * 32 + l31) * LDZ + kh * KD * 16;
            const __bf16 *ape = S::SWZ ? apr + (fsw << 3) : apr + 8 * h, *apo = S::SWZ ? apr + ((fsw ^ 2) << 3) : apr + 8 * h + 16;
#pragma unroll
            for (int kk = 0; kk < KD; ++kk) {
                const __bf16 *ap = ((kk & 1) ? apo : ape) + (kk >> 1) * 32;
                const bf16x8 a0 = *reinterpret_cast<const bf16x8 *>(ap);
                const bf16x8 a1 = *reinterpret_cast<const bf16x8 *>(ap + ZPL);
                const bf16x8 a2 = *reinterpret_cast<const bf16x8 *>(ap + 2 * ZPL);
                acc = __builtin_amdgcn_mfma_f32_32x32x16_bf16(a0, wf[kk][2], acc, 0, 0, 0);
                acc = __builtin_amdgcn_mfma_f32_32x32x16_bf16(a2, wf[kk][0], acc, 0, 0, 0);
                acc = __builtin_amdgcn_mfma_f32_32x32x16_bf16(a1, wf[kk][1], acc, 0, 0, 0);
                acc = __builtin_amdgcn_mfma_f32_32x32x16_bf16(a0, wf[kk][1], acc, 0, 0, 0);
                acc = __builtin_amdgcn_mfma_f32_32x32x16_bf16(a1, wf[kk][0], acc, 0, 0, 0);
                acc = __builtin_amdgcn_mfma_f32_32x32x16_bf16(a0, wf[kk][0], acc, 0, 0, 0);
            }
            if (it == 1) SN_TL(1);
            if (kSkew) __syncthreads();
            if (KS == 2) {
                float *Tx = Tf + (dwv | 1) * (32 * 36);
                if (kh == 1)
#pragma unroll
                    for (int e = 0; e < 16; ++e) Tx[e * 64 + lane] = acc[e];
                __syncthreads();
                if (kh == 0)
#pragma unroll
                    for (int e = 0; e < 16; ++e) acc[e] += Tx[e * 64 + lane];
            }
            if (kh == 0) {
                if (RZ1) {
#pragma clang fp contract(off)
                    const float4 wd = W3s[cb * 32 + l31];
                    const float w3d0 = wd.x, w3d1 = wd.y, w3d2 = wd.z, b3d = wd.w;
                    const float *xq = Xs + (it & 1) * (3 * TR) + rb * 32 + 4 * h;
#pragma unroll
                    for (int q = 0; q < 4; ++q) {
                        const float4 x0 = *reinterpret_cast<const float4 *>(xq + 8 * q);
                        const float4 x1 = *reinterpret_cast<const float4 *>(xq + TR + 8 * q);
                        const float4 x2 = *reinterpret_cast<const float4 *>(xq + 2 * TR + 8 * q);
                        zq[4 * q + 0] = fmaf(w3d2, x2.x, fmaf(w3d1, x1.x, w3d0 * x0.x)) + b3d;
                        zq[4 * q + 1] = fmaf(w3d2, x2.y, fmaf(w3d1, x1.y, w3d0 * x0.y)) + b3d;
                        zq[4 * q + 2] = fmaf(w3d2, x2.z, fmaf(w3d1, x1.z, w3d0 * x0.z)) + b3d;
                        zq[4 * q + 3] = fmaf(w3d2, x2.w, fmaf(w3d1, x1.w, w3d0 * x0.w)) + b3d;
                    }
                }
#pragma unroll
                for (int e = 0; e < 16; ++e) {
                    if (DM == 1) {
// ... 917 lines not shown
}

static DzSrc make_dz(int mode, const float *dy, const float *z, const float *kcoef, const float *gsel, const int *argsel,
                     int rows, int ch, int npts)
{
    DzSrc d{};
    d.mode = mode, d.dy = dy, d.z = z, d.rows = rows, d.ch = ch, d.npts = npts > 0 ? npts : 1;
    d.k1 = kcoef, d.k2 = kcoef ? kcoef + ch : nullptr, d.k3 = kcoef ? kcoef + 2 * ch : nullptr;
    d.gsel = gsel, d.argsel = argsel;
    return d;
}

template <int ZMODE, int PMODE>
static void launch_dgrad(const DgradArgs &g, hipStream_t st)
{
    const int R = g.dz.rows, Ci = g.w.ci, Co = g.w.co;
    if (R <= 32) {
        if (Co % 64 == 0)
            hipLaunchKernelGGL((small_dgrad_kernel<ZMODE, PMODE, true>), dim3((Ci + 31) / 32), dim3(256), 0, st, g);
        else
            hipLaunchKernelGGL((small_dgrad_kernel<ZMODE, PMODE, false>), dim3((Ci + 31) / 32), dim3(256), 0, st, g);
    } else if (R > 64) {
        dim3 grid((R + TileBig::BM - 1) / TileBig::BM, (Ci + TileBig::BN - 1) / TileBig::BN);
        const bool full = R % TileBig::BM == 0 && Ci % TileBig::BN == 0 && Co % BK == 0;
        SN_LAUNCH_T(linear_dgrad_kernel, TileBig, full, grid, g, ZMODE, PMODE);
    } else {
        dim3 grid((R + TileSmall::BM - 1) / TileSmall::BM, (Ci + TileSmall::BN - 1) / TileSmall::BN);
        const bool full = R % TileSmall::BM == 0 && Ci % TileSmall::BN == 0 && Co % BK == 0;
        SN_LAUNCH_T(linear_dgrad_kernel, TileSmall, full, grid, g, ZMODE, PMODE);
    }
}

extern "C" int sn_linear_dgrad(int R, int Ci, int Co, int dz_mode, const float *dy, const float *z, const float *kcoef,
                               const float *gsel, const int *argsel, int npts, const float *W, const float *zprev,
                               const float *coef_prev, float *dyprev, float *stats, sn_stream_t stream)
{
    SN_REQUIRE(R >= 1 && Ci >= 1 && Co >= 1, "bad size");
    SN_REQUIRE(W && dyprev, "null pointer");
    SN_REQUIRE(dz_mode >= DZ_PLAIN && dz_mode <= DZ_POOL, "bad dz_mode");
    DgradArgs g{};
    g.dz = make_dz(dz_mode, dy, z, kcoef, gsel, argsel, R, Co, npts);
    g.w.w = W, g.w.co = Co, g.w.ci = Ci;
    g.prev = make_act(zprev, coef_prev, R, Ci);
    g.dyprev = dyprev, g.stats = stats;
    hipStream_t st = (hipStream_t)stream;
    const bool pm = coef_prev != nullptr;
    if (dz_mode == DZ_PLAIN) {
        if (pm) launch_dgrad<DZ_PLAIN, ACT_BN_RELU>(g, st); else launch_dgrad<DZ_PLAIN, ACT_NONE>(g, st);
    } else if (dz_mode == DZ_BN) {
        if (pm) launch_dgrad<DZ_BN, ACT_BN_RELU>(g, st); else launch_dgrad<DZ_BN, ACT_NONE>(g, st);
    } else {
        if (pm) launch_dgrad<DZ_POOL, ACT_BN_RELU>(g, st); else launch_dgrad<DZ_POOL, ACT_NONE>(g, st);
    }
    SN_LAUNCH_CHECK();
    return 0;
}

static bool conv_bwd_fused_shape(int R, int Ci, int Co)
{
    if (R < 256) return false;
    if ((Ci == 64 && (Co == 64 || Co == 128)) || (Ci == 128 && Co == 128)) return true;
#if SN_BF16X3
    if ((Ci == 128 && Co == 256) || (Ci == 256 && Co == 128)) return true;
#endif
    return false;
}

static int conv_bwd_fused_groups(int R) { return std::min((R + 63) / 64, device_cus()); }

template <int CI, int CO, int ZMODE>
static void launch_conv_bwd_bx3_t(const ConvBwdArgs &a, int G, bool fullr, hipStream_t st)
{
    constexpr size_t lds = CbxShape<CI, CO>::LDS_BYTES;
    static SnLdsAttr at, af;
    (void)sn_lds_attr(at, (const void *)conv_bwd_bx3_kernel<CI, CO, ZMODE, true>, lds, "conv_bwd_bx3_kernel");
    (void)sn_lds_attr(af, (const void *)conv_bwd_bx3_kernel<CI, CO, ZMODE, false>, lds, "conv_bwd_bx3_kernel");
    if (fullr)
        hipLaunchKernelGGL((conv_bwd_bx3_kernel<CI, CO, ZMODE, true>), dim3(G), dim3(512), lds, st, a);
    else
        hipLaunchKernelGGL((conv_bwd_bx3_kernel<CI, CO, ZMODE, false>), dim3(G), dim3(512), lds, st, a);
}

#if SN_BF16X3
template <int ZMODE, int GZ, int GP, int GW, int DM>
static void launch_conv_bwd_bx3_half(const ConvBwdArgs &a, int G, bool fullr, hipStream_t st)
{
    constexpr size_t lds = CbxShape<128, 128>::LDS_BYTES;
    static SnLdsAttr at, af;
    (void)sn_lds_attr(at, (const void *)conv_bwd_bx3_kernel<128, 128, ZMODE, true, false, false, GZ, GP, GW, DM>, lds, "conv_bwd_bx3_kernel");
    (void)sn_lds_attr(af, (const void *)conv_bwd_bx3_kernel<128, 128, ZMODE, false, false, false, GZ, GP, GW, DM>, lds, "conv_bwd_bx3_kernel");
    if (fullr)
        hipLaunchKernelGGL((conv_bwd_bx3_kernel<128, 128, ZMODE, true, false, false, GZ, GP, GW, DM>), dim3(G), dim3(512), lds, st, a);
    else
        hipLaunchKernelGGL((conv_bwd_bx3_kernel<128, 128, ZMODE, false, false, false, GZ, GP, GW, DM>), dim3(G), dim3(512), lds, st, a);
}
#endif

template <int CI, int CO, int ZMODE>
static void launch_conv_bwd_fused_t(const ConvBwdArgs &a, int G, bool fullr, hipStream_t st)
{
#if SN_BF16X3
    launch_conv_bwd_bx3_t<CI, CO, ZMODE>(a, G, fullr, st);
    return;
#endif
    constexpr size_t lds = CbfShape<CI, CO>::LDS_BYTES;
    static SnLdsAttr at, af;
    (void)sn_lds_attr(at, (const void *)conv_bwd_fused_kernel<CI, CO, ZMODE, true>, lds, "conv_bwd_fused_kernel");
    (void)sn_lds_attr(af, (const void *)conv_bwd_fused_kernel<CI, CO, ZMODE, false>, lds, "conv_bwd_fused_kernel");
    if (fullr)
        hipLaunchKernelGGL((conv_bwd_fused_kernel<CI, CO, ZMODE, true>), dim3(G), dim3(512), lds, st, a);
    else
        hipLaunchKernelGGL((conv_bwd_fused_kernel<CI, CO, ZMODE, false>), dim3(G), dim3(512), lds, st, a);
}

static int launch_conv_bwd_fused(int R, int Ci, int Co, int dz_mode, const float *dy, const float *z, const float *kcoef,
                                 const float *gsel, const int *argsel, int npts, const float *W, const float *zprev,
                                 const float *coef_prev, float *dyprev, float *stats, float *part, hipStream_t st,
                                 const ConvBwdArgs *fx = nullptr)
{
    ConvBwdArgs a{};
    if (fx) a.acc_in = fx->acc_in, a.bb_in = fx->bb_in, a.acc_out = fx->acc_out, a.zero_ptr = fx->zero_ptr, a.zero_n = fx->zero_n;
    a.dz.mode = dz_mode, a.dz.dy = dy, a.dz.z = z, a.dz.rows = R, a.dz.ch = Co, a.dz.npts = npts > 0 ? npts : 1;
    a.dz.k1 = kcoef, a.dz.k2 = kcoef ? kcoef + Co : nullptr, a.dz.k3 = kcoef ? kcoef + 2 * Co : nullptr;
    a.dz.gsel = gsel, a.dz.argsel = argsel;
    a.W = W, a.zprev = zprev, a.scale_prev = coef_prev, a.shift_prev = coef_prev + Ci;
    a.dyprev = dyprev, a.stats = stats, a.part = part;
#if SN_BF16X3
    const int TR = Co == 128 ? 32 : 64;
#else
    const int TR = (Ci == 128 && Co == 128) ? 32 : 64;
#endif
    a.ntiles = (R + TR - 1) / TR;
    const int G = conv_bwd_fused_groups(R);
    const bool fullr = R % TR == 0;
#if SN_BF16X3
    if (Co == 256 || Ci == 256) {
        a.ntiles = (R + 31) / 32;
        const bool f32 = R % 32 == 0;
        for (int hh = 0; hh < 2; ++hh) {
            ConvBwdArgs b = a;
            if (Co == 256) {
                b.dz.z = z + 128 * hh, b.dz.dy = dy + 128 * hh, b.dz.ch = 128;
                b.dz.k1 = kcoef + 128 * hh, b.dz.k2 = kcoef + 256 + 128 * hh, b.dz.k3 = kcoef + 512 + 128 * hh;
                b.W = W + (size_t)128 * hh * 128;
                b.part = part + (size_t)128 * hh * 128, b.part_wg_stride = 256 * 128, b.part_ld = 128;
                b.dyacc = dyprev;
                if (hh == 0) launch_conv_bwd_bx3_half<DZ_BN, 256, 128, 128, 1>(b, G, f32, st);
                else launch_conv_bwd_bx3_half<DZ_BN, 256, 128, 128, 2>(b, G, f32, st);
            } else {
                b.W = W + 128 * hh, b.zprev = zprev + 128 * hh, b.dyprev = dyprev + 128 * hh;
                b.scale_prev = coef_prev + 128 * hh, b.shift_prev = coef_prev + 256 + 128 * hh;
                b.stats = stats + 128 * hh, b.stats_ld = 256;
                b.part = part + 128 * hh, b.part_wg_stride = 128 * 256, b.part_ld = 256;
                if (dz_mode == DZ_BN) launch_conv_bwd_bx3_half<DZ_BN, 128, 256, 256, 0>(b, G, f32, st);
                else launch_conv_bwd_bx3_half<DZ_POOL, 128, 256, 256, 0>(b, G, f32, st);
            }
        }
        return G;
    }
#endif
#define SN_CBF(CI_, CO_)                                                                       \
    do {                                                                                       \
        if (dz_mode == DZ_BN) launch_conv_bwd_fused_t<CI_, CO_, DZ_BN>(a, G, fullr, st);        \
        else launch_conv_bwd_fused_t<CI_, CO_, DZ_POOL>(a, G, fullr, st);                       \
    } while (0)
    if (Ci == 64 && Co == 64) SN_CBF(64, 64);
    else if (Ci == 64 && Co == 128) SN_CBF(64, 128);
    else SN_CBF(128, 128);
#undef SN_CBF
    return G;
}

static bool conv_bwd_fused_ok(int R, int Ci, int Co, int dz_mode, int npts, const float *coef_prev, const float *kcoef,
                              const float *db)
{
    return !db && coef_prev && kcoef && conv_bwd_fused_shape(R, Ci, Co) &&
           (dz_mode == DZ_BN || (dz_mode == DZ_POOL && npts > 0 && npts % 64 == 0 && Co != 256));
}

extern "C" int sn_linear_wgrad_splits(int R, int Ci, int Co, int with_bias)
{
    if (R <= 32) return 1;
    if (!with_bias && conv_bwd_fused_shape(R, Ci, Co)) return conv_bwd_fused_groups(R);
    const int ncols = Ci + (with_bias ? 1 : 0);
    const int tiles = ((Co + TileW::BM - 1) / TileW::BM) * ((ncols + TileW::BN - 1) / TileW::BN);
    const int want = std::max(1, 512 / tiles);
    const int maxsplit = std::max(1, (R + 2 * BK - 1) / (2 * BK));
    return std::max(1, std::min(want, maxsplit));
}

template <int ZMODE, int PMODE>
static void launch_wgrad(WgradArgs &g, int R, int Ci, int Co, int with_bias, float *dW, float *db, hipStream_t st)
{
    if (R <= 32) {
        const int tm = (Co + 31) / 32, tn = (g.ncols + 31) / 32;
        hipLaunchKernelGGL((small_wgrad_kernel<ZMODE, PMODE>), dim3((tm * tn + 3) / 4), dim3(256), 0, st, g, dW, db, tn,
                           tm * tn);
        return;
    }
    const int nsplit = sn_linear_wgrad_splits(R, Ci, Co, with_bias);
    int rps = (R + nsplit - 1) / nsplit;
    rps = ((rps + BK - 1) / BK) * BK;
    g.rows_per_split = rps;
    if (ZMODE == DZ_BN && PMODE == ACT_NONE && Ci == 3 && !with_bias) {
        hipLaunchKernelGGL(conv_in3_wgrad_kernel, dim3(nsplit, (Co + 63) / 64), dim3(256), 0, st, R, Co, rps, g.prev.z, g.dz.dy,
                           g.dz.z, g.dz.k1, g.part);
        hipLaunchKernelGGL(wgrad_reduce_kernel, dim3((Co * 3 + 63) / 64), dim3(1024), 0, st, nsplit, Co, 3, 3, g.part, dW, db);
        return;
    }
    dim3 grid((Co + TileW::BM - 1) / TileW::BM, (g.ncols + TileW::BN - 1) / TileW::BN, nsplit);
    const bool full = !with_bias && Co % TileW::BM == 0 && Ci % TileW::BN == 0 && R % rps == 0;
    SN_LAUNCH_T(linear_wgrad_kernel, TileW, full, grid, g, ZMODE, PMODE);
    const int tot = Co * g.ncols;
    hipLaunchKernelGGL(wgrad_reduce_kernel, dim3((tot + 63) / 64), dim3(1024), 0, st, nsplit, Co, Ci, g.ncols, g.part, dW, db);
}

extern "C" int sn_linear_wgrad(int R, int Ci, int Co, int dz_mode, const float *dy, const float *z, const float *kcoef,
                               const float *gsel, const int *argsel, int npts, const float *aprev,
                               const float *coef_prev, float *part, float *dW, float *db, sn_stream_t stream)
{
    SN_REQUIRE(R >= 1 && Ci >= 1 && Co >= 1, "bad size");
    SN_REQUIRE(aprev && part && dW, "null pointer");
    SN_REQUIRE(dz_mode >= DZ_PLAIN && dz_mode <= DZ_POOL, "bad dz_mode");
    const int with_bias = db != nullptr;
    WgradArgs g{};
    g.dz = make_dz(dz_mode, dy, z, kcoef, gsel, argsel, R, Co, npts);
    g.prev = make_act(aprev, coef_prev, R, Ci, with_bias ? Ci : -1);
    g.ncols = Ci + with_bias;
    g.part = part;
    hipStream_t st = (hipStream_t)stream;
    const bool pm = coef_prev != nullptr;
    if (dz_mode == DZ_PLAIN) {
        if (pm) launch_wgrad<DZ_PLAIN, ACT_BN_RELU>(g, R, Ci, Co, with_bias, dW, db, st);
        else launch_wgrad<DZ_PLAIN, ACT_NONE>(g, R, Ci, Co, with_bias, dW, db, st);
    } else if (dz_mode == DZ_BN) {
        if (pm) launch_wgrad<DZ_BN, ACT_BN_RELU>(g, R, Ci, Co, with_bias, dW, db, st);
        else launch_wgrad<DZ_BN, ACT_NONE>(g, R, Ci, Co, with_bias, dW, db, st);
    } else {
        if (pm) launch_wgrad<DZ_POOL, ACT_BN_RELU>(g, R, Ci, Co, with_bias, dW, db, st);
        else launch_wgrad<DZ_POOL, ACT_NONE>(g, R, Ci, Co, with_bias, dW, db, st);
    }
// ... 159 lines not shown
#undef SN_SB
        SN_LAUNCH_CHECK();
        return 0;
    }
    SN_REQUIRE(part, "scratch missing");
    if (conv_bwd_fused_ok(R, Ci, Co, dz_mode, npts, coef_prev, kcoef, db)) {
        SN_REQUIRE(z && (dz_mode != DZ_BN || dy) && (dz_mode != DZ_POOL || (gsel && argsel)), "null pointer");
        const int G = launch_conv_bwd_fused(R, Ci, Co, dz_mode, dy, z, kcoef, gsel, argsel, npts, W, zprev, coef_prev, dyprev,
                                            stats, part, st);
        const int nred = (Co * Ci) % 4 == 0 ? (Co * Ci + kRedElems - 1) / kRedElems : (Co * Ci + 63) / 64;
        hipLaunchKernelGGL(post_bwd_kernel, dim3(nred + (Ci + kChan - 1) / kChan), dim3(1024), 0, st, nred, G, Co, Ci, part, dW,
                           G, Ci, stats, bb);
        SN_LAUNCH_CHECK();
        return 0;
    }
    if (rows_bwd_shape(R, dz_mode)) {
        SN_REQUIRE((dz_mode == DZ_PLAIN || z) && dy, "null pointer");
        const bool fin = coef_prev && R <= 64;
        const int nb = launch_rows_bwd(R, Ci, Co, dz_mode, dy, z, kcoef, W, zprev, coef_prev, dyprev, fin ? nullptr : stats, dW, db, st,
                                       fin ? &bb : nullptr);
        if (coef_prev && !fin)
            hipLaunchKernelGGL(bn_bwd_coef_kernel, dim3((Ci + kChan - 1) / kChan), dim3(1024), 0, st, nb, Ci, stats, bb);
        SN_LAUNCH_CHECK();
        return 0;
    }
    const int nsplit = sn_linear_wgrad_splits(R, Ci, Co, db ? 1 : 0);
    int rps = (R + nsplit - 1) / nsplit;
    rps = ((rps + BK - 1) / BK) * BK;
    const bool plain_top = dz_mode == DZ_PLAIN && dy != nullptr;
    const bool fast = (plain_top || (!db && dz_mode != DZ_PLAIN)) && coef_prev && R % TileBig::BM == 0 && Ci % TileBig::BN == 0 &&
                      Co % BK == 0 && Co % TileW::BM == 0 && Ci % TileW::BN == 0 && R % rps == 0;
    const int nblk = sn_linear_stats_blocks(R);
    if (!fast) {
        int rc = sn_linear_wgrad(R, Ci, Co, dz_mode, dy, z, kcoef, gsel, argsel, npts, zprev, coef_prev, part, dW, db, stream);
        if (rc) return rc;
        rc = sn_linear_dgrad(R, Ci, Co, dz_mode, dy, z, kcoef, gsel, argsel, npts, W, zprev, coef_prev, dyprev, stats, stream);
        if (rc) return rc;
        if (coef_prev)
            hipLaunchKernelGGL(bn_bwd_coef_kernel, dim3((Ci + kChan - 1) / kChan), dim3(1024), 0, st, nblk, Ci, stats, bb);
        SN_LAUNCH_CHECK();
        return 0;
    }
    DgradArgs d{};
    d.dz = make_dz(dz_mode, dy, z, kcoef, gsel, argsel, R, Co, npts);
    d.w.w = W, d.w.co = Co, d.w.ci = Ci;
    d.prev = make_act(zprev, coef_prev, R, Ci);
    d.dyprev = dyprev, d.stats = stats;
    WgradArgs w{};
    w.dz = d.dz;
    w.prev = make_act(zprev, coef_prev, R, Ci, -1);
    w.ncols = Ci, w.part = part, w.rows_per_split = rps;
    const int wgx = Co / TileW::BM, wgy = Ci / TileW::BN, n_w = wgx * wgy * nsplit;
    const int dgx = R / TileBig::BM, n_d = dgx * (Ci / TileBig::BN);
    const dim3 grid(n_w + n_d);
    const size_t lds = shaped_lds(std::max(lds_bytes<TileBig>(), lds_bytes<TileW>()), grid);
    if (dz_mode == DZ_BN)
        hipLaunchKernelGGL((linear_bwd_kernel<TileBig, DZ_BN, ACT_BN_RELU>), grid, dim3(TileBig::THREADS), lds, st, d, w, n_w, wgx, wgy, dgx);
    else if (dz_mode == DZ_POOL)
        hipLaunchKernelGGL((linear_bwd_kernel<TileBig, DZ_POOL, ACT_BN_RELU>), grid, dim3(TileBig::THREADS), lds, st, d, w, n_w, wgx, wgy, dgx);
    else
        hipLaunchKernelGGL((linear_bwd_kernel<TileBig, DZ_PLAIN, ACT_BN_RELU>), grid, dim3(TileBig::THREADS), lds, st, d, w, n_w, wgx, wgy, dgx);
    const int nred = (Co * Ci) % 4 == 0 ? (Co * Ci + kRedElems - 1) / kRedElems : (Co * Ci + 63) / 64;
    const int ndb = db ? (Co + 63) / 64 : 0;
    hipLaunchKernelGGL(post_bwd_kernel, dim3(nred + (Ci + kChan - 1) / kChan + ndb), dim3(1024), 0, st, nred, nsplit, Co, Ci, part, dW, dgx,
                       Ci, stats, bb, dy, R, db);
    SN_LAUNCH_CHECK();
    return 0;
}

extern "C" long long sn_layer_backward_in3_stats_floats(int R, int Ci, int Co)
{
    if (R < 1 || !(Ci == 64 && Co == 64) || !conv_bwd_fused_shape(R, Ci, Co)) return 0;
    return (long long)conv_bwd_fused_groups(R) * 6 * Ci;
}

static void launch_conv_bwd_in3(int R, const float *dy, const float *z, const float *kcoef, const float *W, const float *zprev,
                                const float *coef_prev, float *stats, float *part, const float *x_in, hipStream_t st,
                                const ConvBwdArgs *fx = nullptr, const float *w_in = nullptr, const float *b_in = nullptr)
{
    constexpr int Ci = 64, Co = 64;
    ConvBwdArgs a{};
    a.w_in = w_in, a.b_in = b_in;
    if (fx) a.acc_in = fx->acc_in, a.bb_in = fx->bb_in, a.acc_out = nullptr, a.zero_ptr = fx->zero_ptr, a.zero_n = fx->zero_n;
    a.dz.mode = DZ_BN, a.dz.dy = dy, a.dz.z = z, a.dz.rows = R, a.dz.ch = Co, a.dz.npts = 1;
    a.dz.k1 = kcoef, a.dz.k2 = kcoef ? kcoef + Co : nullptr, a.dz.k3 = kcoef ? kcoef + 2 * Co : nullptr;
    a.W = W, a.zprev = zprev, a.scale_prev = coef_prev, a.shift_prev = coef_prev + Ci;
    a.dyprev = nullptr, a.stats = stats, a.part = part, a.xin = x_in;
    constexpr int TR = CbfShape<64, 64>::TR;
    static_assert(TR == CbxShape<64, 64>::TR, "same tiling in both kernels");
    a.ntiles = (R + TR - 1) / TR;
    const int G = conv_bwd_fused_groups(R);
#if SN_BF16X3
#define SN_CBF_IN3 conv_bwd_bx3_kernel
    constexpr size_t lds = CbxShape<64, 64>::LDS_BYTES_IN3;
    if (!zprev) {
        static SnLdsAttr rt, rf;
        (void)sn_lds_attr(rt, (const void *)conv_bwd_bx3_kernel<64, 64, DZ_BN, true, true, true>, lds, "conv_bwd_bx3_kernel");
        (void)sn_lds_attr(rf, (const void *)conv_bwd_bx3_kernel<64, 64, DZ_BN, false, true, true>, lds, "conv_bwd_bx3_kernel");
        if (R % TR == 0)
            hipLaunchKernelGGL((conv_bwd_bx3_kernel<64, 64, DZ_BN, true, true, true>), dim3(G), dim3(512), lds, st, a);
        else
            hipLaunchKernelGGL((conv_bwd_bx3_kernel<64, 64, DZ_BN, false, true, true>), dim3(G), dim3(512), lds, st, a);
        return;
    }
#else
#define SN_CBF_IN3 conv_bwd_fused_kernel
    constexpr size_t lds = CbfShape<64, 64>::LDS_BYTES_IN3;
#endif
    static SnLdsAttr at, af;
    (void)sn_lds_attr(at, (const void *)SN_CBF_IN3<64, 64, DZ_BN, true, true>, lds, "conv_bwd (xyz layer below)");
    (void)sn_lds_attr(af, (const void *)SN_CBF_IN3<64, 64, DZ_BN, false, true>, lds, "conv_bwd (xyz layer below)");
    if (R % TR == 0)
        hipLaunchKernelGGL((SN_CBF_IN3<64, 64, DZ_BN, true, true>), dim3(G), dim3(512), lds, st, a);
    else
        hipLaunchKernelGGL((SN_CBF_IN3<64, 64, DZ_BN, false, true>), dim3(G), dim3(512), lds, st, a);
#undef SN_CBF_IN3
}

extern "C" int sn_layer_backward_in3(int R, int Ci, int Co, const float *dy, const float *z, const float *kcoef, const float *W,
                                     const float *zprev, const float *coef_prev, float *stats, float *part,
                                     float *dW, float *prev_dgamma, float *prev_dbeta, float *prev_dbias, float *prev_kcoef,
                                     const float *x_in, const float *W_in, const float *b_in, float *dW_in, sn_stream_t stream)
{
    SN_REQUIRE(sn_layer_backward_in3_stats_floats(R, Ci, Co) > 0, "shape not supported by the input-layer variant");
    SN_REQUIRE(dy && z && kcoef && W && zprev && coef_prev && stats && part && dW, "null pointer");
    SN_REQUIRE(prev_dgamma && prev_dbeta && prev_kcoef && x_in && W_in && dW_in, "null pointer");
    hipStream_t st = (hipStream_t)stream;
    launch_conv_bwd_in3(R, dy, z, kcoef, W, zprev, coef_prev, stats, part, x_in, st);
    const int G = conv_bwd_fused_groups(R);
    const BnBwd bb{coef_prev, prev_dgamma, prev_dbeta, prev_dbias, prev_kcoef, (long long)R};
    const int nred = (Co * Ci + kRedElems - 1) / kRedElems;
    hipLaunchKernelGGL(post_bwd_in3_kernel, dim3(nred + (Ci + kChan - 1) / kChan), dim3(1024), 0, st, nred, G, Co, Ci, part, dW, G,
                       Ci, stats, bb, W_in, b_in, dW_in, MultiRed{}, StepTail{});
    SN_LAUNCH_CHECK();
    return 0;
}

static bool conv_stack_backward_ok(int B, int N, int nlayers, const int *ch)
{
    if (!sn_conv_stack_forward_supported(B, N, nlayers, ch) || nlayers < 3 || nlayers > 5) return false;
    const int R = B * N;
    if (ch[1] != 64 || ch[2] != 64 || R < 256) return false;
    for (int l = 1; l < nlayers; ++l)
        if (ch[l] > 128 || ch[l + 1] > 128 || !conv_bwd_fused_shape(R, ch[l], ch[l + 1])) return false;
    return true;
}

extern "C" long long sn_conv_stack_backward_scratch_floats(int B, int N, int nlayers, const int *channels)
{
    if (!conv_stack_backward_ok(B, N, nlayers, channels)) return 0;
    const long long R = (long long)B * N, G = conv_bwd_fused_groups((int)R);
    long long n = 0;
    for (int l = 1; l < nlayers; ++l) n += G * channels[l] * channels[l + 1];
    for (int l = 2; l < nlayers; ++l) n += R * channels[l];
    n += G * 6 * 64 + 3 * 64;
    return n;
}

extern "C" int sn_conv_stack_backward(int B, int N, int nlayers, const int *channels, const float *x, const float *const *W,
                                      const float *bias0, const float *const *z, const float *const *coef, const float *gsel,
                                      const int *argsel, const float *kcoef_top, long long *acc, float *scratch,
                                      float *const *dW, float *const *dgamma, float *const *dbeta, float *const *dbias,
                                      const void *step_tail, sn_stream_t stream)
{
    if (!conv_stack_backward_ok(B, N, nlayers, channels))
        return sn_set_error(SN_ERR_UNSUPPORTED, "sn_conv_stack_backward: shape not supported (use the per-layer entries)");
    SN_REQUIRE(x && W && z && coef && gsel && argsel && kcoef_top && acc && scratch && dW && dgamma && dbeta && dbias, "null pointer");
    for (int l = 0; l < nlayers; ++l) SN_REQUIRE(W[l] && (z[l] || l == 0) && coef[l] && dW[l], "null pointer");
    for (int l = 0; l + 1 < nlayers; ++l) SN_REQUIRE(dgamma[l] && dbeta[l] && dbias[l], "null pointer");
#if !SN_BF16X3
    SN_REQUIRE(z[0], "z[0] == NULL needs the split-bf16 build");
#endif
    hipStream_t st = (hipStream_t)stream;
    const int R = B * N, G = conv_bwd_fused_groups(R);
    const int *ch = channels;
    float *part[5] = {}, *dy[5] = {};
    float *p = scratch;
    for (int l = 1; l < nlayers; ++l) part[l] = p, p += (size_t)G * ch[l] * ch[l + 1];
    for (int l = 2; l < nlayers; ++l) dy[l - 1] = p, p += (size_t)R * ch[l];
    float *stats0 = p;
    p += (size_t)G * 6 * 64;
    float *kcoef0 = p;
    auto accb = [&](int l) { return acc + (size_t)l * kFxLayer; };
    for (int L = nlayers - 1; L >= 1; --L) {
        const int Ci = ch[L], Co = ch[L + 1];
        ConvBwdArgs fx{};
        const bool top = L == nlayers - 1;
        if (!top) {
            fx.acc_in = accb(L);
            fx.bb_in = BnBwd{coef[L], dgamma[L], dbeta[L], dbias[L], nullptr, (long long)R};
            if (L + 1 <= nlayers - 2) fx.zero_ptr = accb(L + 1), fx.zero_n = kFxLayer;
        }
        if (L >= 2) {
            fx.acc_out = accb(L - 1);
            launch_conv_bwd_fused(R, Ci, Co, top ? DZ_POOL : DZ_BN, top ? nullptr : dy[L], z[L], top ? kcoef_top : nullptr,
                                  top ? gsel : nullptr, top ? argsel : nullptr, N, W[L], z[L - 1], coef[L - 1], dy[L - 1], nullptr,
                                  part[L], st, &fx);
        } else {
            launch_conv_bwd_in3(R, dy[1], z[1], nullptr, W[1], z[0], coef[0], stats0, part[1], x, st, &fx, W[0], bias0);
        }
    }
    MultiRed mr{};
    mr.n = nlayers - 1;
    int nb = 0;
    for (int l = 1; l < nlayers; ++l) {
        mr.first[l - 1] = nb, mr.part[l - 1] = part[l], mr.dW[l - 1] = dW[l], mr.elems[l - 1] = ch[l] * ch[l + 1];
        nb += (ch[l] * ch[l + 1] + kRedElems - 1) / kRedElems;
    }
    mr.first[nlayers - 1] = nb;
    mr.zero_ptr = accb(1), mr.zero_n = kFxLayer;
    const BnBwd bb0{coef[0], dgamma[0], dbeta[0], dbias[0], kcoef0, (long long)R};
    StepTail tail{};
    if (step_tail) memcpy(&tail, step_tail, sizeof(tail));
    hipLaunchKernelGGL(post_bwd_in3_kernel, dim3(nb + (64 + kChan - 1) / kChan + (tail.nparts > 0 ? 2 : 0)), dim3(1024), 0, st, nb, G,
                       64, 64, part[1], dW[1], G, 64, stats0, bb0, W[0], bias0, dW[0], mr, tail);
    SN_LAUNCH_CHECK();
    return 0;
}

extern "C" int sn_bn_backward_coef(int nblk, int C, long long R, const float *stats, const float *coef, float *dgamma,
                                   float *dbeta, float *dbias, float *kcoef, sn_stream_t stream)
{
    SN_REQUIRE(nblk >= 1 && C >= 1 && R >= 1 && stats && coef && dgamma && dbeta && kcoef, "bad argument");
    const BnBwd bb{coef, dgamma, dbeta, dbias, kcoef, R};
    hipLaunchKernelGGL(bn_bwd_coef_kernel, dim3((C + kChan - 1) / kChan), dim3(1024), 0, (hipStream_t)stream, nblk, C, stats, bb);
    SN_LAUNCH_CHECK();
    return 0;
}

extern "C" int sn_pool_backward(int B, int C, const float *g, const float *pooled, const float *zsel, float *gsel,
                                float *stats, sn_stream_t stream)
{
    SN_REQUIRE(B >= 1 && C >= 1 && g && pooled && zsel && gsel && stats, "bad argument");
    hipLaunchKernelGGL(pool_bwd_kernel, dim3((C + 63) / 64), dim3(1024), 0, (hipStream_t)stream, B, C, g, pooled, zsel,
                       gsel, stats, BnBwd{});
    SN_LAUNCH_CHECK();
    return 0;
}

extern "C" int sn_pool_backward_bn(int B, int C, long long R, const float *g, const float *pooled, const float *zsel,
                                   float *gsel, const float *coef, float *dgamma, float *dbeta, float *dbias, float *kcoef,
                                   sn_stream_t stream)
{
    SN_REQUIRE(B >= 1 && C >= 1 && R != 0 && g && pooled && zsel && gsel && coef && dgamma && dbeta && kcoef, "bad argument");
    const BnBwd bb{coef, dgamma, dbeta, dbias, kcoef, R};
    hipLaunchKernelGGL(pool_bwd_kernel, dim3((C + 63) / 64), dim3(1024), 0, (hipStream_t)stream, B, C, g, pooled, zsel,
                       gsel, (float *)nullptr, bb);
    SN_LAUNCH_CHECK();
    return 0;
}
```

### samplenet_amd/pointnet.py

```python
import ctypes

import torch

from ._lib import check, lib, ptr, stream_of

DZ_PLAIN, DZ_BN, DZ_POOL = 0, 1, 2
SYNC_STRIDE = 32


def _st(t):
    return stream_of(t)


def _empty(shape, like, dtype=torch.float32):
    return torch.empty(shape, device=like.device, dtype=dtype)


def _arr(ts):
    return (ctypes.c_void_p * len(ts))(*[ptr(t) for t in ts])


def _pool_bufs(B, C, like):
    return _empty((B, C), like), _empty((B, C), like, torch.int32), _empty((B, C), like)

# ... 91 lines not shown
        check(lib.sn_linear_forward_rows(R, L.Ci, L.Co, ptr(a_in), ptr(coef_prev), ptr(L.W), ptr(L.b), ptr(z), _st(a_in)),
              "sn_linear_forward_rows")
        return z, None, 0
    nblk = lib.sn_linear_stats_blocks(R)
    stats = _empty((nblk, 2, L.Co), a_in) if want_stats else None
    check(lib.sn_linear_forward(R, L.Ci, L.Co, ptr(a_in), ptr(coef_prev), ptr(L.W), ptr(L.b), ptr(z), ptr(stats), _st(a_in)),
          "sn_linear_forward")
    return z, stats, nblk


def _momentum(bn):
    if bn.momentum is not None:
        return float(bn.momentum)
    if not bn.track_running_stats or bn.num_batches_tracked is None:
        return 0.0
    return 1.0 / (float(bn.num_batches_tracked.item()) + 1.0)


def _bn_args(bn, update, momentum=None):
    run = (ptr(bn.running_mean), ptr(bn.running_var), ptr(bn.num_batches_tracked)) if update else (None, None, None)
    return (ptr(bn.weight), ptr(bn.bias), float(bn.eps), _momentum(bn) if momentum is None else momentum) + run


def _layer_fwd_bn(R, L, a_in, coef_prev):
    z = _empty((R, L.Co), a_in)
    coef = _empty((4, L.Co), a_in)
    stats = _empty((lib.sn_linear_stats_blocks(R), 2, L.Co), a_in)
    check(lib.sn_layer_forward_bn(R, L.Ci, L.Co, ptr(a_in), ptr(coef_prev), ptr(L.W), ptr(L.b), ptr(z), ptr(stats),
                                  *_bn_args(L.bn, L.bn.track_running_stats), ptr(coef), _st(a_in)), "sn_layer_forward_bn")
    return z, coef


def _layer_fwd_bn_pool(R, npts, L, a_in, coef_prev, pooled, argsel, zsel):
    z = _empty((R, L.Co), a_in)
    coef = _empty((4, L.Co), a_in)
    nblk = lib.sn_linear_stats_blocks(R)
    stats = _empty((nblk, 2, L.Co), a_in)
    pool_val = _empty((nblk, 2, L.Co), a_in)
    pool_idx = _empty((nblk, 2, L.Co), a_in, torch.int32)
    check(lib.sn_conv_forward_bn_pool(R, L.Ci, L.Co, npts, ptr(a_in), ptr(coef_prev), ptr(L.W), ptr(L.b), ptr(z), ptr(stats),
                                      *_bn_args(L.bn, L.bn.track_running_stats), ptr(coef), ptr(pool_val), ptr(pool_idx),
                                      ptr(pooled), ptr(argsel), ptr(zsel), _st(a_in)), "sn_conv_forward_bn_pool")
    return z, coef


def _bn_coef(L, R, stats, nblk, training):
    bn = L.bn
    C = L.Co
    coef = _empty((4, C), L.W)
    if training or not bn.track_running_stats:
        check(lib.sn_bn_finalize(nblk, C, R, ptr(stats), *_bn_args(bn, training and bn.track_running_stats), ptr(coef), _st(L.W)),
              "sn_bn_finalize")
    else:
        check(lib.sn_bn_eval_coef(C, ptr(bn.weight), ptr(bn.bias), float(bn.eps), ptr(bn.running_mean), ptr(bn.running_var),
                                  ptr(coef), _st(L.W)), "sn_bn_eval_coef")
    return coef


def _conv_stack_fwd(convs, x_bnc, training, pool, fuse_pool=False, coef_fn=None):
    B, N, _ = x_bnc.shape
    R = B * N
    a_in, coef = x_bnc.view(R, convs[0].Ci), None
    zs, cs = [], []
    for L in convs:
        if coef_fn is not None:
            z, stats, nblk = _linear_fwd(R, L, a_in, coef, True)
            coef = coef_fn(L, R, stats, nblk)
        elif training and fuse_pool and L is convs[-1]:
            z, coef = _layer_fwd_bn_pool(R, N, L, a_in, coef, *pool)
        elif training:
            z, coef = _layer_fwd_bn(R, L, a_in, coef)
        else:
            z, stats, nblk = _linear_fwd(R, L, a_in, coef, False)
            coef = _bn_coef(L, R, stats, nblk, False)
        zs.append(z)
        cs.append(coef)
        a_in = z
    if not fuse_pool and pool is not None:
        check(lib.sn_pool_forward(B, N, convs[-1].Co, ptr(a_in), ptr(coef), ptr(pool[0]), ptr(pool[1]), ptr(pool[2]), _st(x_bnc)),
              "sn_pool_forward")
    return zs, cs


def _conv_stack_fx(net, convs, x_bnc, B, N, saved, pooled, argsel, zsel, defer_pool=False, rec=None):
    n = len(convs)
    chans = (ctypes.c_int * (n + 1))(convs[0].Ci, *[L.Co for L in convs])
    if any(L.bn.momentum is None or not L.bn.track_running_stats for L in convs):
        return False
    if not lib.sn_conv_stack_forward_supported(B, N, n, chans):
        return False
    if defer_pool and max(chans) > 128:
        return False
    R = B * N
    acc = getattr(net, "_fx_acc", None)
    nacc = lib.sn_conv_stack_acc_elems(n)
    if acc is None or acc.device != x_bnc.device or acc.numel() != nacc:
        acc = torch.zeros(nacc, device=x_bnc.device, dtype=torch.int64)
        net._fx_acc = acc
    zs = [_empty((R, L.Co), x_bnc) for L in convs]
    if Z1_FREE and lib.sn_conv_stack_z1_free_supported(B, N, n, chans):
        zs[0] = None
    cs = [_empty((4, L.Co), x_bnc) for L in convs]
    Cn = convs[-1].Co
    nblk = lib.sn_linear_stats_blocks(R)
    pool_val = _empty((max(nblk, 2 * B) if defer_pool else nblk, 2, Cn), x_bnc)
    pool_idx = _empty((nblk, 2, Cn), x_bnc, torch.int32)
    eps = (ctypes.c_float * n)(*[float(L.bn.eps) for L in convs])
    mom = (ctypes.c_float * n)(*[float(L.bn.momentum) for L in convs])
    args = [B, N, n, chans, ptr(x_bnc), _arr([L.W for L in convs]), _arr([L.b for L in convs]),
            _arr([L.bn.weight for L in convs]), _arr([L.bn.bias for L in convs]),
            _arr([L.bn.running_mean for L in convs]), _arr([L.bn.running_var for L in convs]),
            _arr([L.bn.num_batches_tracked for L in convs]), eps, mom, _arr(zs), _arr(cs), ptr(acc),
            ptr(pool_val), ptr(pool_idx), *([None] * 3 if defer_pool else [ptr(pooled), ptr(argsel), ptr(zsel)]), _st(x_bnc)]
    try:
        check(lib.sn_conv_stack_forward_bn(*args), "sn_conv_stack_forward_bn")
    except Exception:
        acc.zero_()
        raise
    if rec is not None:
        rec.append((lib.sn_conv_stack_forward_bn, "sn_conv_stack_forward_bn", args, 4, acc, (pool_val, pool_idx)))
    saved["zc"], saved["cc"] = zs, cs
    if defer_pool:
        saved["pool_tail"] = (acc, pool_val, pool_idx, convs[-1], n, N, argsel, zsel)
    return True


def _fc_chain_shape(hidden, B):
    n = len(hidden)
    if n < 2 or any(L.bn is None or L.bn.momentum is None or not L.bn.track_running_stats for L in hidden):
        return None
    H, C0 = hidden[0].Co, hidden[0].Ci
    if any(L.Co != H for L in hidden) or any(L.Ci != H for L in hidden[1:]):
        return None
    if not lib.sn_fc_chain_forward_supported(B, C0, H, n):
        return None
    return C0, H, n


def _fc_chain_fwd(net, hidden, pooled, B, saved, rec=None, out=None):
    shape = _fc_chain_shape(hidden, B)
    if shape is None:
        return False
    C0, H, n = shape
    sync = getattr(net, "_fc_sync", None)
    if sync is None or sync.device != pooled.device:
        sync = torch.zeros(16, SYNC_STRIDE, device=pooled.device, dtype=torch.int32)
        net._fc_sync = sync
    xbuf = _empty((2 * 32 * H,), pooled)
    zs = [_empty((B, H), pooled) for _ in hidden]
    cs = [_empty((4, H), pooled) for _ in hidden]
    eps = (ctypes.c_float * n)(*[float(L.bn.eps) for L in hidden])
    mom = (ctypes.c_float * n)(*[float(L.bn.momentum) for L in hidden])
    layer_args = (_arr([L.W for L in hidden]), _arr([L.b for L in hidden]),
                  _arr([L.bn.weight for L in hidden]), _arr([L.bn.bias for L in hidden]),
                  _arr([L.bn.running_mean for L in hidden]), _arr([L.bn.running_var for L in hidden]),
                  _arr([L.bn.num_batches_tracked for L in hidden]), eps, mom, _arr(zs), _arr(cs), ptr(xbuf), ptr(sync), _st(pooled))
    tail = saved.pop("pool_tail", None)
    if tail is not None:
        acc, pool_val, pool_idx, L5, nconv, N, argsel, zsel = tail
        bn5 = L5.bn
        args = [B, N, nconv, ptr(acc), ptr(pool_val), ptr(pool_idx), ptr(bn5.weight), ptr(bn5.bias),
                ptr(bn5.running_mean), ptr(bn5.running_var), ptr(bn5.num_batches_tracked),
                float(bn5.eps), float(bn5.momentum), ptr(saved["cc"][-1]), ptr(pooled), ptr(argsel),
                ptr(zsel), H, n, *layer_args]
        fn, name, keep = lib.sn_fc_chain_forward_pool, "sn_fc_chain_forward_pool", ()
        if out is not None:
            Lo, (_, obn) = out
            if (Lo.Ci == H and obn.momentum is not None and lib.sn_fc_chain_forward_pool_out_supported(B, N, C0, H, n, Lo.Co)):
                upd = obn.track_running_stats
                zo, co, yo = _empty((B, Lo.Co), pooled), _empty((4, Lo.Co), pooled), _empty((B, Lo.Co), pooled)
                args = args[:-1] + [Lo.Co, ptr(Lo.W), ptr(Lo.b), ptr(obn.weight), ptr(obn.bias),
                                    ptr(obn.running_mean) if upd else None, ptr(obn.running_var) if upd else None,
                                    ptr(obn.num_batches_tracked) if upd else None, float(obn.eps), float(obn.momentum),
                                    ptr(zo), ptr(co), ptr(yo), args[-1]]
                fn, name, keep = lib.sn_fc_chain_forward_pool_out, "sn_fc_chain_forward_pool_out", (zo, co, yo)
                saved["z_out"], saved["c_out"], saved["out_fixed"], saved["y_out"] = zo, co, False, yo
        try:
            check(fn(*args), name)
        except Exception:
            acc.zero_()
            raise
        if rec is not None:
            rec.append((fn, name, args, None, acc, keep))
    else:
        check(lib.sn_fc_chain_forward(B, C0, H, n, ptr(pooled), *layer_args), "sn_fc_chain_forward")
    saved["zf"], saved["cf"] = zs, cs
    saved["fc_chain"] = xbuf
    return True


_CHAIN_ERRORS = {1: "forward seam 0", 2: "forward seam 1", 3: "forward seam 2", 64: "epoch hand-over of the backward chain"}


def chain_error_words(net):
    out = []
    for name in ("_fc_sync", "_fc_sync_b"):
        t = getattr(net, name, None)
        out.append(int(t[15, 0].item()) if t is not None else 0)
    return tuple(out)


def check_chain_errors(net, raise_error=True):
    from ._lib import SampleNetHipError

# ... 101 lines not shown

    def __del__(self):
        self.plan.busy = False


class _ForwardPlan:

    kMaxPlans = 4
    __slots__ = ("key", "busy", "calls", "saved", "sig", "last", "captured")

    @staticmethod
    def _signature(net):
        convs, fcs = _layers(net)
        sig = []
        for L in convs + fcs:
            sig += [L.W.data_ptr(), L.b.data_ptr()]
            if L.bn is not None:
                bn = L.bn
                sig += [bn.weight.data_ptr(), bn.bias.data_ptr(), bn.running_mean.data_ptr(), bn.running_var.data_ptr(),
                        bn.num_batches_tracked.data_ptr(), bn.eps, bn.momentum]
        ob = out_bn(net)
        if ob is not None:
            bn = ob[1]
            sig += [bn.weight.data_ptr(), bn.bias.data_ptr(), bn.eps, bn.momentum, bn.track_running_stats] + (
                [bn.running_mean.data_ptr(), bn.running_var.data_ptr(), bn.num_batches_tracked.data_ptr()] if bn.track_running_stats else [])
        return tuple(sig)

    @staticmethod
    def acquire(net, x, skip_last, capturing=False):
        plans = net.__dict__.get("_sn_plans")
        if not plans:
            return None
        key = (x.shape[0], x.shape[1], x.device, bool(skip_last))
        sig = None
        for plan in plans:
            if plan.key == key and not plan.busy and (capturing or not plan.captured):
                if sig is None:
                    sig = _ForwardPlan._signature(net)
                if plan.sig == sig:
                    if capturing and not plan.captured:
                        plan.captured = True
                        net.__dict__.setdefault("_sn_pinned", []).append(plan)
                    return plan
        if sig is not None:
            net.__dict__["_sn_plans"] = [q for q in plans if q.sig == sig or q.key != key]
        return None

    @staticmethod
    def register(net, x, skip_last, rec, saved, last_layer):
        plans = net.__dict__.setdefault("_sn_plans", [])
        if len([q for q in plans if not q.captured]) >= _ForwardPlan.kMaxPlans:
            free = [q for q in plans if not q.busy and not q.captured]
            if not free:
                return
            plans.remove(free[0])
        plan = _ForwardPlan()
        plan.captured = False
        plan.key = (x.shape[0], x.shape[1], x.device, bool(skip_last))
        plan.sig = _ForwardPlan._signature(net)
        plan.calls = rec
        plan.saved = dict(saved)
        plan.saved.pop("_lease", None)
        plan.saved["_bwd_cache"] = saved["_bwd_cache"] = {}
        plan.last = None if ((skip_last and last_layer[1] is None) or "y_out" in saved) else last_layer
        plan.busy = False
        saved["_lease"] = _Lease(plan)
        plans.append(plan)

    def run(self, net, x):
        st = _st(x)
        saved = dict(self.saved)
        saved["x"] = x
        saved["zc"], saved["cc"] = list(saved["zc"]), list(saved["cc"])
        saved["_lease"] = _Lease(self)
        xp = x.data_ptr()
        for fn, name, args, xpos, acc, _keep in self.calls:
            if xpos is not None:
                args[xpos] = xp
            args[-1] = st
            rc = fn(*args)
            if rc != 0:
                acc.zero_()
                check(rc, name)
        y = None
        if self.last is not None:
            y = _last_layer(saved["B"], self.last[0], self.last[1], saved["zf"][-1], saved["cf"][-1], True, saved)
        elif "y_out" in saved:
            y = saved["y_out"] if torch.cuda.is_current_stream_capturing() else saved["y_out"].clone()
        return y, saved


class GradSink(dict):

    def __init__(self, views, params):
        super().__init__(views)
        self.params = params
        self.written = False
        self._reducer_ref = None

    @property
    def reducer(self):
        return self._reducer_ref() if self._reducer_ref is not None else None

    def reset(self):
        self.written = False

    def direct(self):
        return (not self.written) or all(self.params[n].grad is None for n in self)

    def commit(self, fresh=None):
        for n, view in self.items():
            p = self.params[n]
            mine = p.grad is not None and p.grad.data_ptr() == view.data_ptr() and p.grad.shape == view.shape
            if fresh is not None:
                if p.grad is None:
                    view.copy_(fresh[n])
                elif mine:
                    view.add_(fresh[n])
                else:
                    torch.add(p.grad, fresh[n], out=view)
            elif p.grad is not None and not mine:
                view.add_(p.grad)
            if not mine:
                p.grad = view
        self.written = True
        red = getattr(self, "reducer", None)
        if red is not None:
            red._unreduced = True


def sink_for_backward(net):
    sink = getattr(net, "_grad_sink", None)
    if sink is None:
        return None, None
    return (sink if sink.direct() else None), sink


def _out(sink, name, like):
    if sink is not None and name in sink:
        return sink[name]
    return torch.empty_like(like)


FX_STATS = True
IN3_CLOSED_FORM = True
FUSE_POOL = True
Z1_FREE = True
FC_CHAIN = True
POOL_IN_CHAIN = True
FORWARD_PLAN = True


def _wgrad(R, L, mode, dy, z, kcoef, gsel, argsel, npts, aprev, coef_prev, with_bias, sink=None, name=""):
    dW = _out(sink, name + ".weight", L.W)
    db = _out(sink, name + ".bias", L.b) if with_bias else None
    nsplit = lib.sn_linear_wgrad_splits(R, L.Ci, L.Co, 1 if with_bias else 0)
    part = _empty((nsplit * L.Co * (L.Ci + (1 if with_bias else 0)),), L.W)
    check(lib.sn_linear_wgrad(R, L.Ci, L.Co, mode, ptr(dy), ptr(z), ptr(kcoef), ptr(gsel), ptr(argsel), npts, ptr(aprev),
                              ptr(coef_prev), ptr(part), ptr(dW), ptr(db), _st(L.W)), "sn_linear_wgrad")
    return dW, db


def _stats_blocks(nblk, C, like, zero):
    return (torch.zeros if zero else torch.empty)((nblk, 2, C), device=like.device, dtype=torch.float32)


# ... 67 lines not shown
    dbias = _out(sink, L.name + ".bias", L.b)
    kcoef = _empty((3, C), g_pool)
    check(lib.sn_pool_backward_bn(B, C, -1 if fixed else B * saved["N"], ptr(g_pool), ptr(saved["pooled"]), ptr(saved["zsel"]),
                                  ptr(gsel), ptr(saved["cc"][-1]), ptr(dgamma), ptr(dbeta), ptr(dbias), ptr(kcoef), _st(g_pool)),
          "sn_pool_backward_bn")
    grads[L.bn_name + ".weight"], grads[L.bn_name + ".bias"], grads[L.name + ".bias"] = dgamma, dbeta, dbias
    return gsel, kcoef


def _conv_stack_bwd(convs, saved, gsel, kcoef, fixed, grads, sink=None, wgrads=True, input_grad=False, bn_bwd=None, in3=False,
                    dy_top=None):
    B, N = saved["B"], saved["N"]
    R = B * N
    zc, cc, x_rows = saved["zc"], saved["cc"], saved["x"].view(R, convs[0].Ci)
    top = len(convs) - 1
    in3_floats = lib.sn_layer_backward_in3_stats_floats(R, convs[1].Ci, convs[1].Co) if (in3 and convs[0].Ci == 3 and not fixed) else 0
    dy = dy_top
    for i in range(top, 0, -1):
        L, Lp = convs[i], convs[i - 1]
        if i == 1 and in3_floats > 0:
            dW = _out(sink, L.name + ".weight", L.W)
            dW0 = _out(sink, Lp.name + ".weight", Lp.W)
            dg, dbt = _out(sink, Lp.bn_name + ".weight", Lp.bn.weight), _out(sink, Lp.bn_name + ".bias", Lp.bn.bias)
            dbs = _out(sink, Lp.name + ".bias", Lp.b)
            stats = _empty((in3_floats,), L.W)
            part = _empty((lib.sn_linear_wgrad_splits(R, L.Ci, L.Co, 0) * L.Co * L.Ci,), L.W)
            kc = _empty((3, L.Ci), L.W)
            check(lib.sn_layer_backward_in3(R, L.Ci, L.Co, ptr(dy), ptr(zc[1]), ptr(kcoef), ptr(L.W), ptr(_z1(convs, saved)), ptr(cc[0]),
                                            ptr(stats), ptr(part), ptr(dW), ptr(dg), ptr(dbt), ptr(dbs), ptr(kc),
                                            ptr(saved["x"]), ptr(Lp.W), ptr(Lp.b), ptr(dW0), _st(L.W)), "sn_layer_backward_in3")
            grads[L.name + ".weight"], grads[Lp.name + ".weight"] = dW, dW0
            grads[Lp.bn_name + ".weight"], grads[Lp.bn_name + ".bias"], grads[Lp.name + ".bias"] = dg, dbt, dbs
            return None
        mode, gs, ag = (DZ_POOL, gsel, saved["argsel"]) if i == top and dy_top is None else (DZ_BN, None, None)
        zprev = zc[i - 1] if i > 1 else _z1(convs, saved)
        if wgrads and bn_bwd is None:
            dW, _, dy, dg, dbt, dbs, kcoef = _layer_bwd(R, L, mode, dy, zc[i], kcoef, gs, ag, N, zprev, cc[i - 1], Lp, sink, L.name,
                                                        Lp.bn_name, Lp.name, False, -1 if fixed else 0)
            grads[L.name + ".weight"] = dW
            grads[Lp.bn_name + ".weight"], grads[Lp.bn_name + ".bias"], grads[Lp.name + ".bias"] = dg, dbt, dbs
        elif wgrads:
            grads[L.name + ".weight"], dy, stats, _ = _linear_bwd(R, L, mode, dy, zc[i], kcoef, gs, ag, N, zprev, cc[i - 1], sink, True)
            kcoef = bn_bwd(i - 1, stats)
        else:
            dy, stats, nblk = _dgrad(R, L, mode, dy, zc[i], kcoef, gs, ag, N, zprev, cc[i - 1])
            if fixed:
                kcoef = torch.zeros(3, Lp.Co, device=dy.device, dtype=torch.float32)
                kcoef[0].copy_(cc[i - 1][0])
            else:
                kcoef = _bn_bwd(Lp, R, stats, nblk, cc[i - 1])[3]
    L1 = convs[0]
    if wgrads:
        grads[L1.name + ".weight"] = _wgrad(R, L1, DZ_BN, dy, _z1(convs, saved), kcoef, None, None, N, x_rows, None, False, sink, L1.name)[0]
    if input_grad:
        return _dgrad(R, L1, DZ_BN, dy, _z1(convs, saved), kcoef, None, None, N, x_rows, None)[0]
    return None


def conv_stack_backward_supported(net, B, N):
    if not (FX_STATS and IN3_CLOSED_FORM):
        return False
    convs, _ = _layers(net)
    chans = (ctypes.c_int * (len(convs) + 1))(convs[0].Ci, *[L.Co for L in convs])
    return lib.sn_conv_stack_backward_scratch_floats(B, N, len(convs), chans) > 0


def _conv_stack_bwd_fx(net, convs, saved, gsel, kcoef_top, sink, grads, names_c, bn_c, step_tail=None):
    n = len(convs)
    B, N = saved["B"], saved["N"]
    x = saved["x"]
    cache = saved.get("_bwd_cache")
    st = cache.get("conv") if cache is not None else None
    if st is None:
        chans = (ctypes.c_int * (n + 1))(convs[0].Ci, *[L.Co for L in convs])
        nscr = lib.sn_conv_stack_backward_scratch_floats(B, N, n, chans)
        if nscr <= 0:
            return False
        acc = getattr(net, "_fx_acc_b", None)
        nacc = lib.sn_conv_stack_acc_elems(n)
        if acc is None or acc.device != x.device or acc.numel() != nacc:
            acc = torch.zeros(nacc, device=x.device, dtype=torch.int64)
            net._fx_acc_b = acc
        scratch = _empty((nscr,), x)
        st = (chans, acc, scratch, _arr([L.W for L in convs]), _arr(saved["zc"]), _arr(saved["cc"]))
        if cache is not None:
            cache["conv"] = st
    chans, acc, scratch, W_arr, zc_arr, cc_arr = st
    dW = [_out(sink, names_c[i] + ".weight", convs[i].W) for i in range(n)]
    dg = [_out(sink, bn_c[i] + ".weight", convs[i].bn.weight) for i in range(n - 1)]
    dbt = [_out(sink, bn_c[i] + ".bias", convs[i].bn.bias) for i in range(n - 1)]
    dbs = [_out(sink, names_c[i] + ".bias", convs[i].b) for i in range(n - 1)]
    try:
        check(lib.sn_conv_stack_backward(B, N, n, chans, ptr(x), W_arr, ptr(convs[0].b), zc_arr, cc_arr, ptr(gsel),
                                         ptr(saved["argsel"]), ptr(kcoef_top), ptr(acc), ptr(scratch),
                                         _arr(dW), _arr(dg + [None]), _arr(dbt + [None]), _arr(dbs + [None]), step_tail, _st(x)),
              "sn_conv_stack_backward")
    except Exception:
        acc.zero_()
        raise
    for i in range(n):
        grads[names_c[i] + ".weight"] = dW[i]
    for i in range(n - 1):
        grads[bn_c[i] + ".weight"], grads[bn_c[i] + ".bias"], grads[names_c[i] + ".bias"] = dg[i], dbt[i], dbs[i]
    return True


def _fc_chain_bwd(net, convs, fcs, saved, grad_y, sink, grads, fixed, obn=None):
    nf = len(fcs)
    B, R = saved["B"], saved["B"] * saved["N"]
    zf, cf, cc = saved["zf"], saved["cf"], saved["cc"]
    like = grad_y
    L5 = convs[-1]
    C5 = L5.Co
    cache = saved.get("_bwd_cache")
    st = cache.get(("fc", fixed)) if cache is not None else None
    if st is None:
        Co = (ctypes.c_int * nf)(*[fcs[j].Co for j in range(nf - 1, -1, -1)])
        Ci = (ctypes.c_int * nf)(*[fcs[j].Ci for j in range(nf - 1, -1, -1)])
        if nf > 5 or not lib.sn_fc_chain_backward_supported(B, nf, Co, Ci):
            return False
        sync = getattr(net, "_fc_sync_b", None)
        if sync is None or sync.device != like.device:
            sync = torch.zeros(16, SYNC_STRIDE, device=like.device, dtype=torch.int32)
            net._fc_sync_b = sync
        st = {"Co": Co, "Ci": Ci, "sync": sync, "xbuf": _empty((nf * 32 * 256,), like), "gsel": _empty((B, C5), like),
              "kcoef": _empty((3, C5), like)}
        if cache is not None:
            cache[("fc", fixed)] = st
    Co, Ci, sync, xbuf, gsel, kcoef = st["Co"], st["Ci"], st["sync"], st["xbuf"], st["gsel"], st["kcoef"]
    W, zprev, coefprev, rows, dg, dbt, dbs, dW, aprev, araw = [], [], [], [], [], [], [], [], [], []
    keep = []
    for j in range(nf - 1, -1, -1):
        L = fcs[j]
        W.append(L.W)
        dW.append(_out(sink, L.name + ".weight", L.W))
        grads[L.name + ".weight"] = dW[-1]
        if j > 0:
            Lp = fcs[j - 1]
            zprev.append(zf[j - 1]), coefprev.append(cf[j - 1]), aprev.append(zf[j - 1]), araw.append(0)
            rows.append(-1 if (fixed or Lp.bn is None) else B)
            if Lp.bn is not None:
                dg.append(_out(sink, Lp.bn_name + ".weight", Lp.bn.weight)), dbt.append(_out(sink, Lp.bn_name + ".bias", Lp.bn.bias))
                grads[Lp.bn_name + ".weight"], grads[Lp.bn_name + ".bias"] = dg[-1], dbt[-1]
            else:
                dg.append(_empty((Lp.Co,), like)), dbt.append(_empty((Lp.Co,), like))
                keep += [dg[-1], dbt[-1]]
            dbs.append(_out(sink, Lp.name + ".bias", Lp.b))
            grads[Lp.name + ".bias"] = dbs[-1]
        else:
            zprev.append(saved["zsel"]), coefprev.append(cc[-1]), aprev.append(saved["pooled"]), araw.append(1)
            rows.append(-1 if fixed else R)
            dg.append(_out(sink, L5.bn_name + ".weight", L5.bn.weight)), dbt.append(_out(sink, L5.bn_name + ".bias", L5.bn.bias))
            dbs.append(_out(sink, L5.name + ".bias", L5.b))
            grads[L5.bn_name + ".weight"], grads[L5.bn_name + ".bias"], grads[L5.name + ".bias"] = dg[-1], dbt[-1], dbs[-1]
    db_top = _out(sink, fcs[-1].name + ".bias", fcs[-1].b)
    grads[fcs[-1].name + ".bias"] = db_top
    ins = st.get("ins")
    if ins is None:
        ins = (_arr(W), _arr(zprev), _arr(coefprev), (ctypes.c_longlong * nf)(*rows), _arr(aprev), (ctypes.c_int * nf)(*araw))
        st["ins"] = ins
    if obn is not None:
        check(lib.sn_fc_chain_backward_obn(B, nf, Co, Ci, ptr(grad_y), ptr(obn[0]), ptr(obn[1]), int(obn[2]), ptr(obn[3]), ptr(obn[4]),
                                           ins[0], ins[1], ins[2], ins[3], _arr(dg), _arr(dbt), _arr(dbs), _arr(dW), ptr(db_top), ins[4],
                                           ins[5], ptr(gsel), ptr(kcoef), ptr(xbuf), ptr(sync), _st(like)), "sn_fc_chain_backward_obn")
    else:
        check(lib.sn_fc_chain_backward(B, nf, Co, Ci, ptr(grad_y), ins[0], ins[1], ins[2], ins[3],
                                       _arr(dg), _arr(dbt), _arr(dbs), _arr(dW), ptr(db_top), ins[4], ins[5],
                                       ptr(gsel), ptr(kcoef), ptr(xbuf), ptr(sync), _st(like)), "sn_fc_chain_backward")
    saved["fc_chain_b"] = (xbuf, keep)
    return gsel, kcoef


def backward_impl(net, saved, grad_y, sink=None, after_fc=None, step_tail=None):
    convs, fcs = _layers(net)
    names_c, bn_c = [L.name for L in convs], [L.bn_name for L in convs]
    names_f, bn_f = [L.name for L in fcs], [L.bn_name for L in fcs]
    nf = len(fcs)
    B, N = saved["B"], saved["N"]
    R = B * N
# ... 108 lines not shown
```

Baseline: 183,700 point-clouds/s.

## Precompute transposed bf16x3 weight planes in forward for conv backward

The forward weight-split kernel now also writes a transposed, 16-column-tiled copy of each conv layer's bf16x3 weight planes into the accumulator buffer. The backward conv kernels gain a WT template variant that loads these pre-split planes as bf16x8 vectors instead of gathering fp32 weights with strided loads and splitting them per block. The cost being removed is that per-block weight gather and split in every backward workgroup. In exchange the forward kernel does extra strided reads and writes, the accumulator buffer grows, and Python-side version checks guard against stale planes.

New measurement: 182,400 point-clouds/s. About the same (-0.7%).

```diff
diff --git a/include/samplenet_hip_internal.h b/include/samplenet_hip_internal.h
--- a/include/samplenet_hip_internal.h
+++ b/include/samplenet_hip_internal.h
@@ -68,6 +68,7 @@
 long long sn_conv_stack_acc_elems(int nlayers);
 int sn_conv_stack_z1_free_supported(int B, int N, int nlayers, const int *channels);
 long long sn_conv_stack_acc_sum_elems(int nlayers, const int *channels);
+long long sn_conv_stack_wplanes_t_offset(int B, int N, int nlayers, const int *channels, int layer);
 int sn_conv_stack_forward_bn(int B, int N, int nlayers, const int *channels, const float *x, const float *const *W,
                              const float *const *bias, const float *const *gamma, const float *const *beta,
                              float *const *running_mean, float *const *running_var, long long *const *num_batches_tracked,
@@ -79,6 +80,11 @@
                            const int *argsel, const float *kcoef_top, long long *acc, float *scratch, float *const *dW,
                            float *const *dgamma, float *const *dbeta, float *const *dbias, const void *step_tail,
                            sn_stream_t stream);
+int sn_conv_stack_backward_wt(int B, int N, int nlayers, const int *channels, const float *x, const float *const *W,
+                              const float *bias0, const float *const *z, const float *const *coef, const float *gsel,
+                              const int *argsel, const float *kcoef_top, long long *acc, float *scratch, float *const *dW,
+                              float *const *dgamma, float *const *dbeta, float *const *dbias, const void *step_tail,
+                              const void *wplanes_t, sn_stream_t stream);
 int sn_layer_backward(int R, int Ci, int Co, int dz_mode, const float *dy, const float *z, const float *kcoef,
                       const float *gsel, const int *argsel, int npts, const float *W, const float *zprev,
                       const float *coef_prev, float *dyprev, float *stats, float *part, float *dW, float *db,
diff --git a/samplenet_amd/_lib.py b/samplenet_amd/_lib.py
--- a/samplenet_amd/_lib.py
+++ b/samplenet_amd/_lib.py
@@ -93,6 +93,8 @@
     "sn_conv_stack_acc_sum_elems": [_i, ctypes.c_void_p],
     "sn_conv_stack_backward_scratch_floats": [_i, _i, _i, _vp],
     "sn_conv_stack_backward": [_i, _i, _i] + [_vp] * 17,
+    "sn_conv_stack_backward_wt": [_i, _i, _i] + [_vp] * 18,
+    "sn_conv_stack_wplanes_t_offset": [_i, _i, _i, _vp, _i],
     "sn_conv_stack_forward_bn": [_i, _i, _i] + [_vp] * 20,
     "sn_layer_backward_in3_stats_floats": [_i, _i, _i],
     "sn_layer_backward_in3": [_i, _i, _i] + [_vp] * 17 + [_vp],
@@ -171,6 +173,7 @@
              "sn_layer_backward_in3_stats_floats": ctypes.c_longlong,
              "sn_conv_stack_acc_elems": ctypes.c_longlong,
              "sn_conv_stack_acc_sum_elems": ctypes.c_longlong,
+             "sn_conv_stack_wplanes_t_offset": ctypes.c_longlong,
              "sn_conv_stack_backward_scratch_floats": ctypes.c_longlong}
 
 
diff --git a/samplenet_amd/csrc/pointnet_mlp.hip b/samplenet_amd/csrc/pointnet_mlp.hip
--- a/samplenet_amd/csrc/pointnet_mlp.hip
+++ b/samplenet_amd/csrc/pointnet_mlp.hip
@@ -901,7 +901,9 @@
 struct WSplitJob {
     const float *w[4];
     __bf16 *dst[4];
+    __bf16 *dstT[4];
     int elems[4];
+    int ci[4];
     int first[5];
     int n;
     unsigned long long *zero_keys;
@@ -916,6 +918,13 @@
     const int e = (blk - job.first[l]) * 1024 + tid * 4;
     if (e >= job.elems[l]) return;
     const float4 v = *reinterpret_cast<const float4 *>(job.w[l] + e);
+    const bool tr = job.dstT[l] != nullptr;
+    const int Ci = job.ci[l], nr = 1024 / Ci;
+    const int c = tid % Ci, co4 = (blk - job.first[l]) * nr + (tid / Ci) * 4;
+    float ft[4] = {0.f, 0.f, 0.f, 0.f};
+    if (tr)
+#pragma unroll
+        for (int t = 0; t < 4; ++t) ft[t] = job.w[l][(size_t)(co4 + t) * Ci + c];
     bf16x4 p1, p2, p3;
     const float f[4] = {v.x, v.y, v.z, v.w};
 #pragma unroll
@@ -928,6 +937,17 @@
     *reinterpret_cast<bf16x4 *>(d) = p1;
     *reinterpret_cast<bf16x4 *>(d + job.elems[l]) = p2;
     *reinterpret_cast<bf16x4 *>(d + 2 * (size_t)job.elems[l]) = p3;
+    if (!tr) return;
+#pragma unroll
+    for (int t = 0; t < 4; ++t) {
+        __bf16 h1, h2, h3;
+        split3(ft[t], h1, h2, h3);
+        p1[t] = h1, p2[t] = h2, p3[t] = h3;
+    }
+    __bf16 *dt = job.dstT[l] + (size_t)(co4 / 16) * (Ci * 16) + c * 16 + co4 % 16;
+    *reinterpret_cast<bf16x4 *>(dt) = p1;
+    *reinterpret_cast<bf16x4 *>(dt + job.elems[l]) = p2;
+    *reinterpret_cast<bf16x4 *>(dt + 2 * (size_t)job.elems[l]) = p3;
 }
 
 __global__ void __launch_bounds__(256) conv_in3_fwd_kernel(int R, int Co, const float *__restrict__ x,
@@ -1540,9 +1560,23 @@
     if (nlayers <= 0) return 0;
     return (long long)nlayers * ((channels && conv_stack_wide(nlayers, channels)) ? 2 : 1) * kFxLayer;
 }
+static long long conv_stack_planes_end(int nlayers) { return (long long)nlayers * 2 * kFxLayer + (long long)(nlayers - 1) * kWPlaneWideLL; }
 extern "C" long long sn_conv_stack_acc_elems(int nlayers)
 {
-    return nlayers > 0 ? (long long)nlayers * 2 * kFxLayer + (long long)(nlayers - 1) * kWPlaneWideLL : 0;
+    return nlayers > 0 ? conv_stack_planes_end(nlayers) + (long long)(nlayers - 1) * kWPlaneLL : 0;
+}
+extern "C" long long sn_conv_stack_wplanes_t_offset(int B, int N, int nlayers, const int *channels, int layer)
+{
+#if SN_BF16X3
+    if (!sn_conv_stack_forward_supported(B, N, nlayers, channels) || nlayers - 1 > 4 || layer < 1 || layer >= nlayers) return 0;
+    if (conv_stack_wide(nlayers, channels)) return 0;
+    long long nb = 0;
+    for (int l = 1; l < nlayers; ++l) nb += ((long long)channels[l] * channels[l + 1] + 1023) / 1024;
+    if (nb > (long long)B * N / 64) return 0;
+    return conv_stack_planes_end(nlayers) + (long long)(layer - 1) * kWPlaneLL;
+#else
+    return 0;
+#endif
 }
 
 static int g_persist_min_tiles = 4;
@@ -1604,7 +1638,9 @@
         for (int l = 1; l < nlayers; ++l) {
             const int li = l - 1, el = channels[l] * channels[l + 1];
             planes[l] = base + (size_t)li * (wide ? kWPlaneWideLL : kWPlaneLL) * 4;
-            job.w[li] = W[l], job.dst[li] = planes[l], job.elems[li] = el, job.first[li] = nb;
+            job.w[li] = W[l], job.dst[li] = planes[l], job.elems[li] = el, job.ci[li] = channels[l], job.first[li] = nb;
+            const long long offT = sn_conv_stack_wplanes_t_offset(B, N, nlayers, channels, l);
+            job.dstT[li] = offT > 0 ? reinterpret_cast<__bf16 *>(acc + offT) : nullptr;
             nb += (el + 1023) / 1024;
         }
         job.n = nlayers - 1, job.first[job.n] = nb;
diff --git a/samplenet_amd/csrc/pointnet_mlp_backward.hip b/samplenet_amd/csrc/pointnet_mlp_backward.hip
--- a/samplenet_amd/csrc/pointnet_mlp_backward.hip
+++ b/samplenet_amd/csrc/pointnet_mlp_backward.hip
@@ -178,6 +178,7 @@
     int zero_n;
     int part_wg_stride, part_ld, stats_ld;
     const float *dyacc;
+    const __bf16 *wt;
 };
 
 __device__ __forceinline__ float4 buf_load4(sn_rsrc r, unsigned voff, unsigned soff)
@@ -709,9 +710,11 @@
     }
 }
 
-template <int CI, int CO, int ZMODE, bool FULLR, bool IN3 = false, bool RZ1 = false, int GZ = CO, int GP = CI, int GW = CI, int DM = 0>
+template <int CI, int CO, int ZMODE, bool FULLR, bool IN3 = false, bool RZ1 = false, int GZ = CO, int GP = CI, int GW = CI, int DM = 0,
+          bool WT = false>
 __global__ void __launch_bounds__(512) conv_bwd_bx3_kernel(ConvBwdArgs g)
 {
+    static_assert(!WT || (FULLR && DM == 0 && GZ == CO && GP == CI && GW == CI), "WT: whole layers on full tiles (sn_conv_stack_backward_wt)");
     static_assert(DM == 0 || (!IN3 && CbxShape<CI, CO>::KS == 1), "two-pass modes: plain 128 x 128 tiles");
     static_assert(!RZ1 || IN3, "RZ1: the layer below must be the xyz layer");
     using S = CbxShape<CI, CO>;
@@ -761,7 +764,7 @@
         const float scd = g.scale_prev[cb * 32 + l31], shd = g.shift_prev[cb * 32 + l31];
         const unsigned qvo = ((rb * 32 + 4 * h) * GP + cb * 32 + l31) * 4;
         const unsigned ovo = ((rb * 32 + (lane >> 3)) * GP + cb * 32 + (lane & 7) * 4) * 4;
-        const unsigned zvo = ((tid / (CO / 4)) * GZ + zc4) * 4, pvo = ((tid / (CI / 4)) * GP + pc4) * 4, avo = zc4 * 4;
+        const unsigned zvo = ((tid / (CO / 4)) * GZ + zc4) * 4, pvo = WT ? 0u : ((tid / (CI / 4)) * GP + pc4) * 4, avo = zc4 * 4;
         CbfRsrc rs;
         rs.z = make_rsrc(g.dz.z, (unsigned)R * GZ * 4);
         rs.dy = make_rsrc(ZMODE == DZ_BN ? g.dz.dy : g.dz.z, (unsigned)R * GZ * 4);
@@ -801,11 +804,20 @@
         int tile = tile0;
         cbf_issue_loads<CO, CI, TR, ZMODE, NZ4, NP4, true, GZ, GP>(rs, tile, cloud, zvo, pvo, avo, rz, rdy, rp, rag, rgs);
         if (xthr) rx = buf_load4(rsx, (unsigned)tid * 16, (unsigned)tile * (TR * 12));
-        float wraw[KD][8];
-#pragma unroll
-        for (int kk = 0; kk < KD; ++kk)
-#pragma unroll
-            for (int t = 0; t < 8; ++t) wraw[kk][t] = g.W[(size_t)((kh * KD + kk) * 16 + 8 * h + t) * GW + cb * 32 + l31];
+        float wraw[WT ? 1 : KD][8];
+        bf16x8 wf[KD][3];
+        if constexpr (WT) {
+            const __bf16 *wr = g.wt + (size_t)(kh * KD * CI + cb * 32 + l31) * 16 + 8 * h;
+#pragma unroll
+            for (int kk = 0; kk < KD; ++kk)
+#pragma unroll
+                for (int p = 0; p < 3; ++p) wf[kk][p] = *reinterpret_cast<const bf16x8 *>(wr + (size_t)p * (CI * CO) + kk * (CI * 16));
+        } else {
+#pragma unroll
+            for (int kk = 0; kk < KD; ++kk)
+#pragma unroll
+                for (int t = 0; t < 8; ++t) wraw[kk][t] = g.W[(size_t)((kh * KD + kk) * 16 + 8 * h + t) * GW + cb * 32 + l31];
+        }
         if (fxin) {
             const float *Ks = Tf;
             __syncthreads();
@@ -815,15 +827,16 @@
         }
         cbx_stage<CO, CI, TR, ZMODE, FULLR, NZ4>(g, tile, tic * TR, tid, Lb, rz, rdy, rag, rgs, k1, k2, k3);
         if (xthr) Xs[xslot[0]] = rx.x, Xs[xslot[1]] = rx.y, Xs[xslot[2]] = rx.z, Xs[xslot[3]] = rx.w;
-        bf16x8 wf[KD][3];
-#pragma unroll
-        for (int kk = 0; kk < KD; ++kk)
-#pragma unroll
-            for (int t = 0; t < 8; ++t) {
-                __bf16 h1, h2, h3;
-                split3(wraw[kk][t], h1, h2, h3);
-                wf[kk][0][t] = h1, wf[kk][1][t] = h2, wf[kk][2][t] = h3;
-            }
+        if constexpr (!WT) {
+#pragma unroll
+            for (int kk = 0; kk < KD; ++kk)
+#pragma unroll
+                for (int t = 0; t < 8; ++t) {
+                    __bf16 h1, h2, h3;
+                    split3(wraw[kk][t], h1, h2, h3);
+                    wf[kk][0][t] = h1, wf[kk][1][t] = h2, wf[kk][2][t] = h3;
+                }
+        }
         __syncthreads();
         for (int it = 0; tile < tend; ++it, tile += tst) {
             const __bf16 *Zb = Lb + (it & 1) * BUF;
@@ -1907,6 +1920,15 @@
 }
 
 #if SN_BF16X3
+template <int CI, int CO, int ZMODE>
+static void launch_conv_bwd_bx3_wt(const ConvBwdArgs &a, int G, hipStream_t st)
+{
+    constexpr size_t lds = CbxShape<CI, CO>::LDS_BYTES;
+    static SnLdsAttr at;
+    (void)sn_lds_attr(at, (const void *)conv_bwd_bx3_kernel<CI, CO, ZMODE, true, false, false, CO, CI, CI, 0, true>, lds, "conv_bwd_bx3_kernel");
+    hipLaunchKernelGGL((conv_bwd_bx3_kernel<CI, CO, ZMODE, true, false, false, CO, CI, CI, 0, true>), dim3(G), dim3(512), lds, st, a);
+}
+
 template <int ZMODE, int GZ, int GP, int GW, int DM>
 static void launch_conv_bwd_bx3_half(const ConvBwdArgs &a, int G, bool fullr, hipStream_t st)
 {
@@ -1945,6 +1967,7 @@
 {
     ConvBwdArgs a{};
     if (fx) a.acc_in = fx->acc_in, a.bb_in = fx->bb_in, a.acc_out = fx->acc_out, a.zero_ptr = fx->zero_ptr, a.zero_n = fx->zero_n;
+    if (fx) a.wt = fx->wt;
     a.dz.mode = dz_mode, a.dz.dy = dy, a.dz.z = z, a.dz.rows = R, a.dz.ch = Co, a.dz.npts = npts > 0 ? npts : 1;
     a.dz.k1 = kcoef, a.dz.k2 = kcoef ? kcoef + Co : nullptr, a.dz.k3 = kcoef ? kcoef + 2 * Co : nullptr;
     a.dz.gsel = gsel, a.dz.argsel = argsel;
@@ -1982,6 +2005,13 @@
             }
         }
         return G;
+    }
+#endif
+#if SN_BF16X3
+    if (a.wt && fullr) {
+        if (Ci == 128 && Co == 128 && dz_mode == DZ_POOL) return launch_conv_bwd_bx3_wt<128, 128, DZ_POOL>(a, G, st), G;
+        if (Ci == 64 && Co == 128 && dz_mode == DZ_BN) return launch_conv_bwd_bx3_wt<64, 128, DZ_BN>(a, G, st), G;
+        if (Ci == 64 && Co == 64 && dz_mode == DZ_BN) return launch_conv_bwd_bx3_wt<64, 64, DZ_BN>(a, G, st), G;
     }
 #endif
 #define SN_CBF(CI_, CO_)                                                                       \
@@ -2307,6 +2337,7 @@
     ConvBwdArgs a{};
     a.w_in = w_in, a.b_in = b_in;
     if (fx) a.acc_in = fx->acc_in, a.bb_in = fx->bb_in, a.acc_out = nullptr, a.zero_ptr = fx->zero_ptr, a.zero_n = fx->zero_n;
+    if (fx) a.wt = fx->wt;
     a.dz.mode = DZ_BN, a.dz.dy = dy, a.dz.z = z, a.dz.rows = R, a.dz.ch = Co, a.dz.npts = 1;
     a.dz.k1 = kcoef, a.dz.k2 = kcoef ? kcoef + Co : nullptr, a.dz.k3 = kcoef ? kcoef + 2 * Co : nullptr;
     a.W = W, a.zprev = zprev, a.scale_prev = coef_prev, a.shift_prev = coef_prev + Ci;
@@ -2322,7 +2353,11 @@
         static SnLdsAttr rt, rf;
         (void)sn_lds_attr(rt, (const void *)conv_bwd_bx3_kernel<64, 64, DZ_BN, true, true, true>, lds, "conv_bwd_bx3_kernel");
         (void)sn_lds_attr(rf, (const void *)conv_bwd_bx3_kernel<64, 64, DZ_BN, false, true, true>, lds, "conv_bwd_bx3_kernel");
-        if (R % TR == 0)
+        if (a.wt && R % TR == 0) {
+            static SnLdsAttr rw;
+            (void)sn_lds_attr(rw, (const void *)conv_bwd_bx3_kernel<64, 64, DZ_BN, true, true, true, 64, 64, 64, 0, true>, lds, "conv_bwd_bx3_kernel");
+            hipLaunchKernelGGL((conv_bwd_bx3_kernel<64, 64, DZ_BN, true, true, true, 64, 64, 64, 0, true>), dim3(G), dim3(512), lds, st, a);
+        } else if (R % TR == 0)
             hipLaunchKernelGGL((conv_bwd_bx3_kernel<64, 64, DZ_BN, true, true, true>), dim3(G), dim3(512), lds, st, a);
         else
             hipLaunchKernelGGL((conv_bwd_bx3_kernel<64, 64, DZ_BN, false, true, true>), dim3(G), dim3(512), lds, st, a);
@@ -2382,11 +2417,13 @@
     return n;
 }
 
-extern "C" int sn_conv_stack_backward(int B, int N, int nlayers, const int *channels, const float *x, const float *const *W,
-                                      const float *bias0, const float *const *z, const float *const *coef, const float *gsel,
-                                      const int *argsel, const float *kcoef_top, long long *acc, float *scratch,
-                                      float *const *dW, float *const *dgamma, float *const *dbeta, float *const *dbias,
-                                      const void *step_tail, sn_stream_t stream)
+extern "C" long long sn_conv_stack_wplanes_t_offset(int B, int N, int nlayers, const int *channels, int layer);
+
+static int conv_stack_backward(int B, int N, int nlayers, const int *channels, const float *x, const float *const *W,
+                               const float *bias0, const float *const *z, const float *const *coef, const float *gsel,
+                               const int *argsel, const float *kcoef_top, long long *acc, float *scratch,
+                               float *const *dW, float *const *dgamma, float *const *dbeta, float *const *dbias,
+                               const void *step_tail, const void *wplanes_t, sn_stream_t stream)
 {
     if (!conv_stack_backward_ok(B, N, nlayers, channels))
         return sn_set_error(SN_ERR_UNSUPPORTED, "sn_conv_stack_backward: shape not supported (use the per-layer entries)");
@@ -2407,9 +2444,14 @@
     p += (size_t)G * 6 * 64;
     float *kcoef0 = p;
     auto accb = [&](int l) { return acc + (size_t)l * kFxLayer; };
+    const long long wt1 = wplanes_t ? sn_conv_stack_wplanes_t_offset(B, N, nlayers, channels, 1) : 0;
+    SN_REQUIRE(!wplanes_t || wt1 > 0, "wplanes_t: the forward writes no transposed planes for this shape");
     for (int L = nlayers - 1; L >= 1; --L) {
         const int Ci = ch[L], Co = ch[L + 1];
         ConvBwdArgs fx{};
+        if (wplanes_t)
+            fx.wt = reinterpret_cast<const __bf16 *>(static_cast<const long long *>(wplanes_t) +
+                                                     (sn_conv_stack_wplanes_t_offset(B, N, nlayers, channels, L) - wt1));
         const bool top = L == nlayers - 1;
         if (!top) {
             fx.acc_in = accb(L);
@@ -2443,6 +2485,26 @@
     return 0;
 }
 
+extern "C" int sn_conv_stack_backward(int B, int N, int nlayers, const int *channels, const float *x, const float *const *W,
+                                      const float *bias0, const float *const *z, const float *const *coef, const float *gsel,
+                                      const int *argsel, const float *kcoef_top, long long *acc, float *scratch,
+                                      float *const *dW, float *const *dgamma, float *const *dbeta, float *const *dbias,
+                                      const void *step_tail, sn_stream_t stream)
+{
+    return conv_stack_backward(B, N, nlayers, channels, x, W, bias0, z, coef, gsel, argsel, kcoef_top, acc, scratch, dW, dgamma, dbeta,
+                               dbias, step_tail, nullptr, stream);
+}
+
+extern "C" int sn_conv_stack_backward_wt(int B, int N, int nlayers, const int *channels, const float *x, const float *const *W,
+                                         const float *bias0, const float *const *z, const float *const *coef, const float *gsel,
+                                         const int *argsel, const float *kcoef_top, long long *acc, float *scratch,
+                                         float *const *dW, float *const *dgamma, float *const *dbeta, float *const *dbias,
+                                         const void *step_tail, const void *wplanes_t, sn_stream_t stream)
+{
+    return conv_stack_backward(B, N, nlayers, channels, x, W, bias0, z, coef, gsel, argsel, kcoef_top, acc, scratch, dW, dgamma, dbeta,
+                               dbias, step_tail, wplanes_t, stream);
+}
+
 extern "C" int sn_bn_backward_coef(int nblk, int C, long long R, const float *stats, const float *coef, float *dgamma,
                                    float *dbeta, float *dbias, float *kcoef, sn_stream_t stream)
 {
diff --git a/samplenet_amd/pointnet.py b/samplenet_amd/pointnet.py
--- a/samplenet_amd/pointnet.py
+++ b/samplenet_amd/pointnet.py
@@ -197,6 +197,20 @@
     return zs, cs
 
 
+def _wt_record(acc, wt_ptr, Ws):
+    return (acc, wt_ptr, Ws, tuple((W.data_ptr(), W._version) for W in Ws))
+
+
+def _wt_planes(saved):
+    rec = saved.get("wt")
+    if rec is None:
+        return None
+    _acc, wt_ptr, Ws, vers = rec
+    if any((W.data_ptr(), W._version) != v for W, v in zip(Ws, vers)):
+        return None
+    return wt_ptr
+
+
 def _conv_stack_fx(net, convs, x_bnc, B, N, saved, pooled, argsel, zsel, defer_pool=False, rec=None):
     n = len(convs)
     chans = (ctypes.c_int * (n + 1))(convs[0].Ci, *[L.Co for L in convs])
@@ -235,6 +249,9 @@
     if rec is not None:
         rec.append((lib.sn_conv_stack_forward_bn, "sn_conv_stack_forward_bn", args, 4, acc, (pool_val, pool_idx)))
     saved["zc"], saved["cc"] = zs, cs
+    off = lib.sn_conv_stack_wplanes_t_offset(B, N, n, chans, 1)
+    if off > 0:
+        saved["wt"] = _wt_record(acc, acc.data_ptr() + 8 * off, [L.W for L in convs[1:]])
     if defer_pool:
         saved["pool_tail"] = (acc, pool_val, pool_idx, convs[-1], n, N, argsel, zsel)
     return True
@@ -502,6 +519,8 @@
             if rc != 0:
                 acc.zero_()
                 check(rc, name)
+        if "wt" in saved:
+            saved["wt"] = _wt_record(*saved["wt"][:3])
         y = None
         if self.last is not None:
             y = _last_layer(saved["B"], self.last[0], self.last[1], saved["zf"][-1], saved["cf"][-1], True, saved)
@@ -735,19 +754,24 @@
             acc = torch.zeros(nacc, device=x.device, dtype=torch.int64)
             net._fx_acc_b = acc
         scratch = _empty((nscr,), x)
-        st = (chans, acc, scratch, _arr([L.W for L in convs]), _arr(saved["zc"]), _arr(saved["cc"]))
+        st = (chans, acc, scratch, _arr([L.W for L in convs]), _arr(saved["zc"]), _arr(saved["cc"]),
+              saved["wt"][1] if "wt" in saved else None)
         if cache is not None:
             cache["conv"] = st
-    chans, acc, scratch, W_arr, zc_arr, cc_arr = st
+    chans, acc, scratch, W_arr, zc_arr, cc_arr, wt_ptr = st
+    if wt_ptr is not None and _wt_planes(saved) != wt_ptr:
+        wt_ptr = None
     dW = [_out(sink, names_c[i] + ".weight", convs[i].W) for i in range(n)]
     dg = [_out(sink, bn_c[i] + ".weight", convs[i].bn.weight) for i in range(n - 1)]
     dbt = [_out(sink, bn_c[i] + ".bias", convs[i].bn.bias) for i in range(n - 1)]
     dbs = [_out(sink, names_c[i] + ".bias", convs[i].b) for i in range(n - 1)]
+    args = (B, N, n, chans, ptr(x), W_arr, ptr(convs[0].b), zc_arr, cc_arr, ptr(gsel), ptr(saved["argsel"]), ptr(kcoef_top),
+            ptr(acc), ptr(scratch), _arr(dW), _arr(dg + [None]), _arr(dbt + [None]), _arr(dbs + [None]), step_tail)
     try:
-        check(lib.sn_conv_stack_backward(B, N, n, chans, ptr(x), W_arr, ptr(convs[0].b), zc_arr, cc_arr, ptr(gsel),
-                                         ptr(saved["argsel"]), ptr(kcoef_top), ptr(acc), ptr(scratch),
-                                         _arr(dW), _arr(dg + [None]), _arr(dbt + [None]), _arr(dbs + [None]), step_tail, _st(x)),
-              "sn_conv_stack_backward")
+        if wt_ptr is not None:
+            check(lib.sn_conv_stack_backward_wt(*args, wt_ptr, _st(x)), "sn_conv_stack_backward_wt")
+        else:
+            check(lib.sn_conv_stack_backward(*args, _st(x)), "sn_conv_stack_backward")
     except Exception:
         acc.zero_()
         raise
```
